# marcinp7/music-style-transfer

Hardware: AMD Instinct MI355X
Metric: style-transfer opt iters/sec (higher is better)
Workload: dtype f32; 1 GPU; one 30 s clip per GPU (BASELINE.json configs[1]): piano-roll C=4,R=16,T=4 (+percussion), full widths (980325 params), fwd+loss+bwd every step, Adam+StepLR every iter_size steps; clips_per_gpu=1, iter_size=2, hip_graph=True, graphs=one joint graph, accumulation=2 concurrent streams, launches_per_pass=72, parallelism=single GPU

## Files before the change

__graft_entry__.py:

```python
import os
import subprocess
import sys

ROOT = os.path.dirname(os.path.abspath(__file__))
PKG = os.path.join(ROOT, 'music-style-transfer_amd')
CSRC = os.path.join(PKG, 'csrc')
BUILD = os.path.join(PKG, 'build')
LIB = os.path.join(PKG, 'libmst_amd.so')
SOURCES = ['gemm', 'lstm', 'combine', 'notes', 'loss_optim', 'plan', 'audio', 'conv', 'lin']
for p in (ROOT, PKG):
    if p not in sys.path:
        sys.path.insert(0, p)


def _hipcc():
    for c in (os.environ.get('HIPCC'), '/opt/rocm/bin/hipcc', 'hipcc'):
        if c and (os.path.isabs(c) and os.path.exists(c) or not os.path.isabs(c)):
            return c
    raise RuntimeError('hipcc not found')


def _stale(target, deps):
    return not os.path.exists(target) or any(os.path.getmtime(d) > os.path.getmtime(target) for d in deps)


def build(force=False):
    os.makedirs(BUILD, exist_ok=True)
    hipcc = _hipcc()
    headers = [os.path.join(CSRC, 'mst_common.h'), os.path.join(CSRC, 'combine_body.h'), os.path.join(ROOT, 'include', 'mst_amd.h')]
    procs, objs = [], []
    for s in SOURCES:
        src, obj = os.path.join(CSRC, s + '.hip'), os.path.join(BUILD, s + '.o')
        objs.append(obj)
        if force or _stale(obj, [src] + headers):
            cmd = [hipcc, '--offload-arch=gfx950', '-O3', '-std=c++17', '-fPIC', '-c', src, '-o', obj]
            procs.append((s, subprocess.Popen(cmd, stdout=subprocess.PIPE, stderr=subprocess.STDOUT)))
    for s, p in procs:
        out, _ = p.communicate()
        if p.returncode:
            raise RuntimeError(f'hipcc failed on {s}.hip:\n{out.decode()}')
    if force or _stale(LIB, objs):
        subprocess.run([hipcc, '--offload-arch=gfx950', '-shared', '-fPIC', '-o', LIB] + objs, check=True)
    import style
    from style import _native
    _native.Native(LIB)


def smoke():
    import numpy as np
    import torch
    from oracle import style_oracle as so
    from tools.synth import synth_clip
    from style import _native as nat
    if not os.path.exists(LIB):
        build()
    assert torch.cuda.is_available(), 'smoke() needs cuda:0'
    dev = torch.device('cuda:0')
    native = nat.get()
    C, R, T = 2, 2, 4
    dims = nat.Dims(C=C, R=R, T=T, beat=64, bar=128, nrf=8, style=256, melody=8, rhythm=32, instr=51,
                    n_instruments=41, has_unpitched=1)
    table = native.param_table(dims)
    g = torch.Generator().manual_seed(0)
    flat = torch.zeros(native.param_floats(dims))
    named = {}
    for name, off, shape in table:
        n = int(np.prod(shape))
        fan = shape[1] if len(shape) > 1 else shape[0]
        flat[off:off + n] = (torch.rand(n, generator=g) * 2 - 1) / fan ** 0.5
        named[name] = flat[off:off + n].view(*shape).clone().requires_grad_(True)
    clip = synth_clip(5, C, R, T, True)
    _, ref_losses = so.iteration(named, clip)
    plan = native.plan(dims, dev)
    plan.set_inputs(mode=clip['mode'], bpm=clip['bpm'], instr=clip['instruments_features'],
                    used=clip['used_instruments'], bpm_target=float(clip['bpm_int']))
    params = flat.to(dev)
    gparams = torch.zeros_like(params)
    losses = torch.zeros(nat.N_LOSSES, device=dev)
    plan.train_iteration(params, gparams, clip['pitched'].to(dev), clip['unpitched'].to(dev), losses)
    torch.cuda.synchronize()
    got = losses.cpu()
    for i, k in enumerate(nat.LOSS_KEYS):
        assert abs(float(got[i]) - ref_losses[k]) < 1e-4, (k, float(got[i]), ref_losses[k])
    gref = torch.cat([(named[n].grad if named[n].grad is not None else torch.zeros_like(named[n])).reshape(-1)
                      for n, _, _ in table])
    err = float((gparams.cpu() - gref).norm() / gref.norm())
    assert err < 1e-4, err
    print(f'smoke ok: total loss {float(got[0]):.6f} (oracle {ref_losses["total"]:.6f}), grad rel-L2 {err:.2e}')


if __name__ == '__main__':
    build()
    print('built', LIB)
```

include/mst_amd.h:

```cpp
#ifndef MST_AMD_H
#define MST_AMD_H
#include <stdint.h>

#ifdef __cplusplus
extern "C" {
#endif

typedef enum {
    MST_OK = 0,
    MST_ERR_ARG = -1,
    MST_ERR_UNSUPPORTED = -2,
    MST_ERR_LAUNCH = -3,
    MST_ERR_ALLOC = -4,
} mst_status;

typedef struct {
    int32_t C, R, T;
    int32_t beat, bar, nrf;
    int32_t style, melody, rhythm;
    int32_t instr;
    int32_t n_instruments;
    int32_t has_unpitched;
    int32_t clips;
} mst_dims;
// ... 41 lines not shown

int32_t mst_forward(const mst_plan* p, int32_t stage_mask, const float* params, float* ws,
                    const float* pitched, const float* unpitched, mst_stream stream);

int32_t mst_backward(const mst_plan* p, int32_t stage_mask, const float* params, float* gparams,
                     float* ws, const float* pitched, const float* unpitched, mst_stream stream);
int32_t mst_zero_grads(const mst_plan* p, int32_t stage_mask, float* ws, mst_stream stream);
int64_t mst_plan_zero_floats(const mst_plan* p, int32_t stage_mask);

#define MST_LOSS_SAVED 512
int64_t mst_loss_scratch_floats(void);
int32_t mst_total_loss_fwd(const float* pitched_pred, const float* pitched_target, int64_t n_pitched_pos,
                           const float* unpitched_pred, const float* unpitched_target, int64_t n_unpitched_pos,
                           const float* instr_logits, const float* instr_target, int32_t n_instr,
                           const float* mode_logits, const float* mode_target,
                           const float* bpm_pred, const float* bpm_target,
                           int32_t normalize, float* losses, float* saved, float* scratch, mst_stream stream);
int32_t mst_total_loss_bwd(const float* pitched_pred, const float* pitched_target, int64_t n_pitched_pos,
                           const float* unpitched_pred, const float* unpitched_target, int64_t n_unpitched_pos,
                           const float* instr_logits, const float* instr_target, int32_t n_instr,
                           const float* mode_logits, const float* mode_target,
                           const float* bpm_pred, const float* bpm_target,
                           const float* saved, const float* grad_losses,
                           float* g_pitched, float* g_unpitched, float* g_instr, float* g_mode, float* g_bpm,
                           mst_stream stream);

int32_t mst_train_iteration(const mst_plan* p, const float* params, float* gparams, float* ws,
                            const float* pitched, const float* unpitched, float* losses, mst_stream stream);

#define MST_MAX_XCHG 8
int32_t mst_tiled_phase_count(const mst_plan* p);
int32_t mst_tiled_phase(const mst_plan* p, int32_t phase, const float* params, float* gparams, float* ws,
                        const float* pitched, const float* unpitched, float* losses, int32_t is_root,
                        mst_stream stream, int64_t xoff[MST_MAX_XCHG], int64_t xlen[MST_MAX_XCHG], int32_t* nx);

int32_t mst_adam_step(float* params, float* grads, float* exp_avg, float* exp_avg_sq, int64_t n,
                      float* state, double lr0, double beta1, double beta2, double eps,
                      int32_t step_size, double gamma, int32_t zero_grad, mst_stream stream);

int32_t mst_adam_step2(float* params, float* grads, float* grads2, float* exp_avg, float* exp_avg_sq, int64_t n,
                       float* state, double lr0, double beta1, double beta2, double eps,
                       int32_t step_size, double gamma, int32_t zero_grad, mst_stream stream);

#define MST_GUARD_WORDS 8
int64_t mst_grad_guard_scratch_bytes(int64_t n);
int32_t mst_grad_norm(const float* grads, const float* grads2 , int64_t n, void* scratch, float* norm,
                      mst_stream stream);
int32_t mst_grad_norms(const float* grads, const float* grads2 , const int64_t* offsets, const int64_t* lengths,
                       int32_t count, float* norms, mst_stream stream);
int32_t mst_adam_step_guarded(float* params, float* grads, float* grads2 , float* exp_avg, float* exp_avg_sq,
                              int64_t n, float* state, float* guard, void* scratch, double lr0, double beta1, double beta2,
                              double eps, int32_t step_size, double gamma, double max_norm ,
                              int32_t skip_nonfinite, int32_t zero_grad, mst_stream stream);

int32_t mst_hard_output(float* x, float* out, int64_t n_pos, int32_t nfeat, mst_stream stream);

int32_t mst_clip_scatter(const int32_t* cells, const float* feats, const int32_t* counts, int32_t capacity, int32_t n_clips,
                         int64_t n_cells, int32_t nfeat, float* out, mst_stream stream);

typedef struct { int32_t first, count, src_bars, r0; } mst_window;
int32_t mst_clip_window(const int32_t* cells, const float* feats, const mst_window* win, int32_t n_clips, int32_t channels,
                        int32_t bars, int64_t bar_cells, int32_t nfeat, float* out, mst_stream stream);

enum { MST_ROLL_NONZERO = 0, MST_ROLL_HARD = 1 };
int64_t mst_roll_slices(int64_t n_cells);
int32_t mst_roll_count(const float* x, int64_t n_cells, int32_t nfeat, int32_t mode, int32_t* ws, mst_stream stream);
int32_t mst_roll_compact(const float* x, int64_t n_cells, int32_t nfeat, int32_t mode, const int32_t* ws,
                         int64_t capacity, int32_t* cells, float* feats, mst_stream stream);

#define MST_METRIC_WORDS 8
int64_t mst_roll_metrics_scratch_bytes(int64_t n_groups, int64_t group_cells);
int32_t mst_roll_metrics(const float* pred, const float* target, int64_t n_groups, int64_t group_cells,
                         int32_t nfeat, void* scratch, double* out, mst_stream stream);

int64_t mst_eval_scratch_bytes(const mst_plan* p);
int32_t mst_eval_iteration(const mst_plan* p, const float* params, float* ws, const float* pitched,
                           const float* unpitched, float* losses, double* metrics, void* scratch, mst_stream stream);

int32_t mst_plan_step_count(const mst_plan* p, int32_t stage_mask, int32_t backward);
int32_t mst_plan_step_info(const mst_plan* p, int32_t stage_mask, int32_t backward, int32_t* info );
int32_t mst_plan_step_carried(const mst_plan* p, int32_t stage_mask, int32_t backward, int32_t* carried);
int32_t mst_plan_step_riders(const mst_plan* p, int32_t stage_mask, int32_t backward, int32_t* out);
int32_t mst_plan_zero_rides(const mst_plan* p);
int32_t mst_plan_step_gemms(const mst_plan* p, int32_t stage_mask, int32_t backward, int32_t step, int32_t* out, int32_t cap);
int32_t mst_plan_time_steps(const mst_plan* p, int32_t stage_mask, int32_t backward, const float* params,
                            float* gparams, float* ws, const float* pitched, const float* unpitched,
                            mst_stream stream, int32_t reps, float* ms, int32_t* kind, double* flops, double* bytes);

typedef struct mst_audio_plan mst_audio_plan;
mst_audio_plan* mst_audio_plan_create(int32_t n_fft , int32_t hop, int64_t n_samples, int32_t* status);
void mst_audio_plan_destroy(mst_audio_plan* p);
int32_t mst_audio_plan_info(const mst_audio_plan* p, int64_t out[6]);
int32_t mst_audio_stft(const mst_audio_plan* p, const float* audio, float* spec, float* mag, mst_stream stream);
int32_t mst_audio_gram(const mst_audio_plan* p, const float* feat, float* gram, float* ws, mst_stream stream);
int32_t mst_audio_style_iteration(const mst_audio_plan* p, float* x, const float* gram_style, float* grad, float* exp_avg,
                                  float* exp_avg_sq, float* state, float* ws, float* loss, double lr, mst_stream stream);

int32_t mst_debug_slab_columns_disjoint(int64_t off_x, int32_t width_x, int64_t off_y, int32_t width_y, int32_t ld);

const char* mst_version(void);

#ifdef __cplusplus
}
#endif
#endif
```

music-style-transfer_amd/csrc/gemm.hip:

```cpp
#include "combine_body.h"

__device__ __forceinline__ float act_fwd(int act, float z, int col) {
    if (act == ACT_LEAKY) return z > 0.f ? z : z * LEAKY;
    if (act == ACT_SIGOUT) { float s = 1.f / (1.f + expf(-z)); return col == 0 ? 6.f * s : s; }
    if (act == ACT_BPM) { float s = 1.f / (1.f + expf(-z)); return s * 150.f + 50.f; }
    return z;
}

__device__ __forceinline__ float act_bwd(int act, float y, int col) {
    if (act == ACT_LEAKY) return y > 0.f ? 1.f : LEAKY;
    if (act == ACT_SIGOUT) return col == 0 ? y * (1.f - y * (1.f / 6.f)) : y * (1.f - y);
    if (act == ACT_BPM) { float s = (y - 50.f) * (1.f / 150.f); return 150.f * s * (1.f - s); }
    return 1.f;
}

typedef const MST_GLOBAL_AS float* gcptr;
#define GEMM_PAD 1

template <int KIND>
__device__ __forceinline__ int off_of(const Operand& o, int i, int j, bool& ok) {
    if constexpr (KIND == OPK_DENSE) {
        return i * (int)o.si + j * (int)o.sj;
    } else if constexpr (KIND == OPK_ACTGRAD) {
        return o.transposed ? j * o.ld + i : i * o.ld + j;
    } else if constexpr (KIND == OPK_IM2COL) {
        const int p = i >> 3, oc = i & 7;
        const int f = j / (CONV_K * NPF), rem = j - f * (CONV_K * NPF);
        const int e = (NDEG * oc - CONV_PAD) * NPF + rem;
        ok = ok & (e >= 0) & (e < NPN * NPF);
        return p * (NF * NPN * NPF) + f * (NPN * NPF) + e;
    } else if constexpr (KIND == OPK_PERMW) {
        if (o.pb == CONV_K && o.pc == NPF) {
            constexpr int BC = CONV_K * NPF;
            const int a = i / BC, rem = i - a * BC;
            const int bb = rem / NPF, c = rem - bb * NPF;
            return j * o.ld + a * BC + c * CONV_K + bb;
        }
        if (o.pb == NUN && o.pc == NUF) {
            constexpr int BC = NUN * NUF;
            const int a = i / BC, rem = i - a * BC;
            const int bb = rem / NUF, c = rem - bb * NUF;
            return j * o.ld + a * BC + c * NUN + bb;
        }
        const int bc = o.pb * o.pc;
        const int a = i / bc, rem = i - a * bc;
        const int bb = rem / o.pc, c = rem - bb * o.pc;
        return j * o.ld + a * bc + c * o.pb + bb;
    } else {
        return (j >> 3) * (o.oc * NOCT) + i * NOCT + (j & 7);
    }
}

template <int OK>
__device__ __forceinline__ void store_out(const GemmDesc& d, float* cbase, const float* bias, int m, int n, int split, float acc) {
    const OutSpec& o = d.out;
    if constexpr (OK == OUT_STORE) {
        float v = acc;
        if (bias) v += o.bias_div > 0 ? bias[(unsigned)((m / o.bias_div) * o.bias_ld + n)] : bias[n];
        cbase[(unsigned)(m * o.ldc + n)] = act_fwd(o.act, v, n);
    } else if constexpr (OK == OUT_ACCUM) {
        float* c = cbase + (unsigned)(m * o.ldc + n);
        *c = o.first ? acc : *c + acc;
    } else if constexpr (OK == OUT_CONV) {
        cbase[(unsigned)((m >> 3) * o.ldc + n * NOCT + (m & 7))] = act_fwd(ACT_LEAKY, acc + bias[n], 0);
    } else if constexpr (OK == OUT_SLAB) {
        const unsigned idx = n < o.wcols ? (unsigned)(m * o.wcols + n) : (unsigned)(d.M * o.wcols + m);
        cbase[(int64_t)split * o.slab_stride + idx] = acc;
    } else {
        unsigned idx;
        if (n < o.wcols) {
            int a, bb, c, bc;
            if (o.pb == CONV_K && o.pc == NPF) { bc = CONV_K * NPF; a = n / (CONV_K * NPF); const int rem = n - a * (CONV_K * NPF); bb = rem / NPF; c = rem - bb * NPF; }
            else if (o.pb == NUN && o.pc == NUF) { bc = NUN * NUF; a = n / (NUN * NUF); const int rem = n - a * (NUN * NUF); bb = rem / NUF; c = rem - bb * NUF; }
            else { bc = o.pb * o.pc; a = n / bc; const int rem = n - a * bc; bb = rem / o.pc; c = rem - bb * o.pc; }
            idx = (unsigned)(m * o.wcols + a * bc + c * o.pb + bb);
        } else {
            idx = (unsigned)(d.M * o.wcols + m);
        }
        cbase[(int64_t)split * o.slab_stride + idx] = acc;
    }
}

template <int AK, int BKIND, int OK, int AKF, int BKF, int KD>
// ... 473 lines not shown
                    }
                }
            }
            const int n = tn * MF_BN + bn * 32 + (lane & 31);
            if ((ks == 0) & (tm * MF_BM + bm * 32 < M) & (tn * MF_BN + bn * 32 < N)) {
#pragma unroll
                for (int r = 0; r < 16; ++r) {
                    const int m = tm * MF_BM + bm * 32 + (r & 3) + 8 * (r >> 2) + 4 * (lane >> 5);
                    if (m < M && n < N) store_out<OK>(d, cbase, bias, m, n, split, acc[r]);
                }
            }
#pragma unroll
            for (int r = 0; r < 16; ++r) acc[r] = 0.f;
        }
        if (!more) break;
        t = nt; kt = nkt; buf ^= 1;
    }
}

__global__ __launch_bounds__(MF_THREADS, 4) void gemm_mfma_kernel(const GemmDesc* __restrict__ descs, const int* __restrict__ owner, int count, int blocks_per_clip, Bases b) {
    __shared__ float smem[2 * 2 * MF_KD * (MF_BM + GEMM_PAD)];
    float (*As)[MF_BM + GEMM_PAD] = reinterpret_cast<float (*)[MF_BM + GEMM_PAD]>(smem);
    float (*Bs)[MF_BN + GEMM_PAD] = reinterpret_cast<float (*)[MF_BN + GEMM_PAD]>(smem + MF_KD * (MF_BM + GEMM_PAD));
    const int clip = blockIdx.x / blocks_per_clip, lb = blockIdx.x - clip * blocks_per_clip;
    const int lo = owner[lb];
    const GemmDesc d = descs[clip * count + lo];
    const int local = lb - d.blk_begin;
    const int ntile = ((d.M + MF_BM - 1) / MF_BM) * ((d.N + MF_BN - 1) / MF_BN);
    const int run = d.run > 0 ? d.run : 1, nruns = (ntile + run - 1) / run;
    const int split = local / nruns, t_begin = (local - split * nruns) * run, t_end = min(ntile, t_begin + run);
    switch (d.variant) {
    case GV_LIN_FWD: gemm_fast_body<OPK_DENSE, OUT_STORE, 1, 1>(d, b, t_begin, t_end, split, smem); break;
    case GV_LIN_DW: gemm_fast_body<OPK_ACTGRAD, OUT_SLAB, 0, 0>(d, b, t_begin, t_end, split, smem); break;
    case GV_LIN_DW_PERM: gemm_fast_body<OPK_ACTGRAD, OUT_PERMW_SLAB, 0, 0>(d, b, t_begin, t_end, split, smem); break;
    case GV_LIN_DA: gemm_fast_body<OPK_ACTGRAD, OUT_ACCUM, 1, 0>(d, b, t_begin, t_end, split, smem); break;
    case GV_HH_DW: gemm_fast_body<OPK_DENSE, OUT_SLAB, 0, 0>(d, b, t_begin, t_end, split, smem); break;
    case GV_LIN_DA_RAW: gemm_fast_body<OPK_DENSE, OUT_ACCUM, 1, 0>(d, b, t_begin, t_end, split, smem); break;
    default:
        for (int tile = t_begin; tile < t_end; ++tile) {
            if (tile > t_begin) __syncthreads();
            if (d.variant == GV_LIN_FWD_PERM) gemm_mfma_body<OPK_DENSE, OPK_PERMW, OUT_STORE, 1, 1>(d, b, tile, split, As, Bs);
            else if (d.variant == GV_CONV_FWD) gemm_mfma_body<OPK_IM2COL, OPK_PERMW, OUT_CONV, 1, 1>(d, b, tile, split, As, Bs);
            else if (d.variant == GV_CONV_DW) {
                if (d.fold_rows) gemm_mfma_body<OPK_CONVGRAD, OPK_IM2COL, OUT_PERMW_SLAB, 1, 0, true>(d, b, tile, split, As, Bs);
                else gemm_mfma_body<OPK_CONVGRAD, OPK_IM2COL, OUT_PERMW_SLAB, 1, 0>(d, b, tile, split, As, Bs);
            }
        }
        break;
    }
}

int gemm_tile_edge(int mfma) { return mfma ? MF_BM : GEMM_BM; }
int gemm_blocks(const GemmDesc& g, int mfma) {
    const int edge = gemm_tile_edge(mfma);
    const int ntile = ((g.M + edge - 1) / edge) * ((g.N + edge - 1) / edge);
    const int run = (mfma && g.run > 1) ? g.run : 1;
    return ((ntile + run - 1) / run) * g.ksplit;
}

__device__ __forceinline__ void combine_rider(const CombineDesc d, const int cb, int kind, const Bases& b, float* smem) {
    constexpr int ROW = COMBINE_MAXC + 1;
    const int tid = threadIdx.x;
    if ((kind == COMB_RIDE_SUMSQ || kind == COMB_RIDE_REDUCE) && combine_site_small(d)) {
        if (cb != 0) return;
        kind = kind == COMB_RIDE_SUMSQ ? COMB_RIDE_SMALL_F : COMB_RIDE_SMALL_B;
    }
    if (kind == COMB_RIDE_SMALL_F) {
        combine_small_fwd_body<4>(d, tid, tid < 256, b, reinterpret_cast<float (*)[ROW]>(smem), smem + 4 * ROW);
    } else if (kind == COMB_RIDE_SMALL_B) {
        if (d.first) combine_small_bwd_body<4, true>(d, tid, tid < 256, b, smem, smem + ROW, reinterpret_cast<float (*)[ROW]>(smem + 2 * ROW));
        else combine_small_bwd_body<4, false>(d, tid, tid < 256, b, smem, smem + ROW, reinterpret_cast<float (*)[ROW]>(smem + 2 * ROW));
    } else {
        const int gi = tid >> 8, grp = cb * 4 + gi;
        float* slice = smem + gi * 5 * ROW;
        if (kind == COMB_RIDE_SUMSQ) combine_sumsq_body<4>(d, grp, tid & 255, grp < d.nblk, b, reinterpret_cast<float (*)[ROW]>(slice), slice + 4 * ROW);
        else combine_bwd_reduce_body<4>(d, grp, tid & 255, grp < d.nblk, b, reinterpret_cast<float (*)[ROW]>(slice), slice + 4 * ROW);
    }
}

template <int WV> __device__ __forceinline__ void gather_rows(const GatherDesc& d, const int blk, const int nblk, const Bases& b);
__device__ __forceinline__ void segred_group(const SegRedDesc* __restrict__ descs, const int members, const int clip, const int lb, const int t, const Bases& b);

__device__ __forceinline__ void gemm_rider_block(const GemmRiders& r, const int clip, int lb, const Bases& b, float* smem) {
    const int seg_blocks = (r.seg_groups + 3) >> 2, gat_blocks = r.gat_members * r.gat_blocks;
#pragma unroll
    for (int q = 0; q < 2; ++q) {
        const GemmRiders::Comb& cr = r.comb[q];
        const int comb_blocks = cr.sites * cr.blocks;
        if (lb < comb_blocks) {
            const int m = lb / cr.blocks;
            combine_rider(cr.descs[clip * cr.sites + m], lb - m * cr.blocks, cr.kind, b, smem);
            return;
        }
        lb -= comb_blocks;
    }
    if (lb < seg_blocks) {
        const int grp = lb * 4 + (threadIdx.x >> 8);
        if (grp < r.seg_groups) segred_group(r.segreds, r.seg_members, clip, grp, threadIdx.x & 255, b);
        return;
    }
    lb -= seg_blocks;
    if (lb < gat_blocks) {
        const int m = lb / r.gat_blocks;
        gather_rows<GATHER_RIDER_ROWS>(r.gathers[clip * r.gat_members + m], lb - m * r.gat_blocks, r.gat_blocks, b);
        return;
    }
    lb -= gat_blocks;
    if (lb < r.zero_chunks) {
        const ZeroChunk c = r.zero[lb];
        float* p = b.p[SP_GRAD] + (int64_t)clip * r.zero_stride + c.off;
        for (int i = threadIdx.x; i < c.len; i += GEMM_THREADS) p[i] = 0.f;
    }
}

__global__ __launch_bounds__(GEMM_THREADS) void gemm_kernel(const GemmDesc* __restrict__ descs, const int* __restrict__ owner, int count, int blocks_per_clip, int rider_blocks, Bases b, GemmRiders r) {
    constexpr int TILE_F = GEMM_BK * (GEMM_BM + GEMM_PAD), RED_F = (GEMM_THREADS / 64) * GEMM_BM * GEMM_BN;
    __shared__ float smem[(2 * TILE_F > RED_F) ? 2 * TILE_F : RED_F];
    float (*As)[GEMM_BM + GEMM_PAD] = reinterpret_cast<float (*)[GEMM_BM + GEMM_PAD]>(smem);
    float (*Bs)[GEMM_BN + GEMM_PAD] = reinterpret_cast<float (*)[GEMM_BN + GEMM_PAD]>(smem + TILE_F);
    const int clip = blockIdx.x / blocks_per_clip;
    int lb = blockIdx.x - clip * blocks_per_clip;
    if (lb < rider_blocks) {
        gemm_rider_block(r, clip, lb, b, smem);
        return;
    }
    lb -= rider_blocks;
    const int lo = owner[lb];
    const GemmDesc d = descs[clip * count + lo];
    const int local = lb - d.blk_begin;
    const int ntile = ((d.M + GEMM_BM - 1) / GEMM_BM) * ((d.N + GEMM_BN - 1) / GEMM_BN);
    const int tile = local % ntile, split = local / ntile;
#define GEMM_CASE(V, A_, B_, O_, AF_, BF_)                                                          \
    case (V) * 3 + 0: gemm_body<A_, B_, O_, AF_, BF_, 32>(d, b, tile, split, As, Bs); break;           \
    case (V) * 3 + 1: gemm_body<A_, B_, O_, AF_, BF_, 64>(d, b, tile, split, As, Bs); break;           \
    case (V) * 3 + 2: gemm_body<A_, B_, O_, AF_, BF_, 128>(d, b, tile, split, As, Bs); break;
    switch (d.variant * 3 + d.kdsel) {
        GEMM_CASE(GV_LIN_FWD, OPK_DENSE, OPK_DENSE, OUT_STORE, 1, 1)
        GEMM_CASE(GV_LIN_FWD_PERM, OPK_DENSE, OPK_PERMW, OUT_STORE, 1, 1)
        GEMM_CASE(GV_LIN_DW, OPK_ACTGRAD, OPK_DENSE, OUT_SLAB, 0, 0)
        GEMM_CASE(GV_LIN_DW_PERM, OPK_ACTGRAD, OPK_DENSE, OUT_PERMW_SLAB, 0, 0)
        GEMM_CASE(GV_LIN_DA, OPK_ACTGRAD, OPK_DENSE, OUT_ACCUM, 1, 0)
        GEMM_CASE(GV_CONV_FWD, OPK_IM2COL, OPK_PERMW, OUT_CONV, 1, 1)
        GEMM_CASE(GV_CONV_DW, OPK_CONVGRAD, OPK_IM2COL, OUT_PERMW_SLAB, 1, 0)
        GEMM_CASE(GV_HH_DW, OPK_DENSE, OPK_DENSE, OUT_SLAB, 0, 0)
        GEMM_CASE(GV_LIN_DA_RAW, OPK_DENSE, OPK_DENSE, OUT_ACCUM, 1, 0)
    default: break;
    }
#undef GEMM_CASE
}

int gemm_variant(const GemmDesc& g) {
    const int a = g.A.kind, bk = g.B.kind, o = g.out.kind;
    if (a == OPK_DENSE && bk == OPK_DENSE && o == OUT_STORE) return GV_LIN_FWD;
    if (a == OPK_DENSE && bk == OPK_PERMW && o == OUT_STORE) return GV_LIN_FWD_PERM;
    if (a == OPK_ACTGRAD && bk == OPK_DENSE && o == OUT_SLAB) return GV_LIN_DW;
    if (a == OPK_ACTGRAD && bk == OPK_DENSE && o == OUT_PERMW_SLAB) return GV_LIN_DW_PERM;
    if (a == OPK_ACTGRAD && bk == OPK_DENSE && o == OUT_ACCUM) return GV_LIN_DA;
    if (a == OPK_IM2COL && bk == OPK_PERMW && o == OUT_CONV) return GV_CONV_FWD;
    if (a == OPK_CONVGRAD && bk == OPK_IM2COL && o == OUT_PERMW_SLAB) return GV_CONV_DW;
    if (a == OPK_DENSE && bk == OPK_DENSE && o == OUT_SLAB) return GV_HH_DW;
    if (a == OPK_DENSE && bk == OPK_DENSE && o == OUT_ACCUM) return GV_LIN_DA_RAW;
    return -1;
}

int gemm_rider_blocks(const GemmRiders& r) { return r.comb[0].sites * r.comb[0].blocks + r.comb[1].sites * r.comb[1].blocks + (r.seg_groups + 3) / 4 + r.gat_members * r.gat_blocks + r.zero_chunks; }

int launch_gemm(const GemmDesc* dev_descs, const int* dev_owner, int members, int blocks_per_clip, int clips, int mfma, Bases b, hipStream_t s, const GemmRiders* riders) {
    if (members <= 0 || blocks_per_clip <= 0 || clips <= 0) return 0;
    GemmRiders r = riders ? *riders : GemmRiders{};
    if (mfma && gemm_rider_blocks(r)) return (int)hipErrorInvalidValue;
    blocks_per_clip += gemm_rider_blocks(r);
    if (mfma) hipLaunchKernelGGL(gemm_mfma_kernel, dim3(blocks_per_clip * clips), dim3(MF_THREADS), 0, s, dev_descs, dev_owner, members, blocks_per_clip, b);
    else hipLaunchKernelGGL(gemm_kernel, dim3(blocks_per_clip * clips), dim3(GEMM_THREADS), 0, s, dev_descs, dev_owner, members, blocks_per_clip, gemm_rider_blocks(r), b, r);
    return (int)hipGetLastError();
}

template <int WV>
__device__ __forceinline__ void gather_rows(const GatherDesc& d, const int blk, const int nblk, const Bases& b) {
    const int lane = threadIdx.x & 63, wv = (threadIdx.x >> 6) & (WV - 1);
    for (int row = blk * WV + wv; row < d.rows; row += nblk * WV) {
        unsigned t = (unsigned)row;
        int rc[4];
        rc[3] = t % (unsigned)d.d[3]; t /= (unsigned)d.d[3];
        rc[2] = t % (unsigned)d.d[2]; t /= (unsigned)d.d[2];
        rc[1] = t % (unsigned)d.d[1]; rc[0] = t / (unsigned)d.d[1];
        float* out = b.p[SP_WS] + d.out_off + (int64_t)row * d.K;
        if (d.sum) {
            for (int w = lane; w < d.K; w += 64) {
                float a = 0.f;
                for (int sIdx = 0; sIdx < d.nseg; ++sIdx) {
                    const Seg& sg = d.seg[sIdx];
                    const int srow = rc[0] * sg.s[0] + rc[1] * sg.s[1] + rc[2] * sg.s[2] + rc[3] * sg.s[3];
                    a += b.p[sg.space][sg.off + (int64_t)srow * sg.ld + w];
                }
                out[w] = a;
            }
            continue;
        }
        for (int sIdx = 0; sIdx < d.nseg; ++sIdx) {
            const Seg& sg = d.seg[sIdx];
            const int srow = rc[0] * sg.s[0] + rc[1] * sg.s[1] + rc[2] * sg.s[2] + rc[3] * sg.s[3];
            const float* src = b.p[sg.space] + sg.off + (int64_t)srow * sg.ld;
            for (int w = lane; w < sg.width; w += 64) out[sg.start + w] = src[w];
        }
    }
}

__global__ __launch_bounds__(256) void gather_kernel(const GatherDesc* __restrict__ descs, Bases b) {
    gather_rows<4>(descs[blockIdx.y], blockIdx.x, gridDim.x, b);
}

int launch_gather(const GatherDesc* dev, int count, int max_rows, Bases b, hipStream_t s) {
    if (count <= 0) return 0;
    int gx = (max_rows + 3) / 4;
    if (gx > 2048) gx = 2048;
    hipLaunchKernelGGL(gather_kernel, dim3(gx, count), dim3(256), 0, s, dev, b);
    return (int)hipGetLastError();
}

#define SEGRED_CHUNK 64
template <int E, int R>
__device__ __forceinline__ void segred_body(const SegRedDesc& d, const int item, const Bases& b) {
    const int wgrp = (d.width + E - 1) / E;
    if (item >= d.nidx * d.nchunk * wgrp) return;
    const int w = (item % wgrp) * E, ne = min(E, d.width - w);
    int t = item / wgrp;
    const int chunk = t % d.nchunk, idx = t / d.nchunk;
    int kc[4];
    t = idx;
#pragma unroll
    for (int q = 3; q >= 0; --q) { kc[q] = t % d.kd[q]; t /= d.kd[q]; }
    int rd[4], nred = 1;
#pragma unroll
    for (int q = 0; q < 4; ++q) { rd[q] = d.kd[q] == 1 ? d.d[q] : 1; nred *= rd[q]; }
    const int r_begin = chunk * SEGRED_CHUNK, r_end = min(nred, r_begin + SEGRED_CHUNK);
    int cr[4];
    t = r_begin;
#pragma unroll
    for (int q = 3; q >= 0; --q) { cr[q] = t % rd[q]; t /= rd[q]; }
    const float* src = b.p[SP_GRAD] + d.src_off + d.start + w;
    const float* ysrc = b.p[SP_WS] + d.y_off + d.start + w;
    const int64_t s3 = d.src_ld, s2 = s3 * d.d[3], s1 = s2 * d.d[2], s0 = s1 * d.d[1];
    const int64_t w3 = s2 - rd[3] * s3, w2 = s1 - rd[2] * s2, w1 = s0 - rd[1] * s1;
    int64_t roff = (kc[0] + cr[0]) * s0 + (kc[1] + cr[1]) * s1 + (kc[2] + cr[2]) * s2 + (kc[3] + cr[3]) * s3;
    auto offset = [&]() { return roff; };
    auto advance = [&]() {
        roff += s3;
        if (++cr[3] == rd[3]) { cr[3] = 0; roff += w3; if (++cr[2] == rd[2]) { cr[2] = 0; roff += w2; if (++cr[1] == rd[1]) { cr[1] = 0; roff += w1; ++cr[0]; } } }
// ... 162 lines not shown
```

music-style-transfer_amd/csrc/lstm.hip:

```cpp
#include "mst_common.h"

#define LSTM_ZS 8192
#define LSTM_MCH 32
__device__ __forceinline__ float sigm(float x) { return MST_FAST_RCP(1.f + MST_FAST_EXP(-x)); }
__device__ __forceinline__ float tanh_fast(float x) { return 2.f * sigm(2.f * x) - 1.f; }
__device__ __forceinline__ float wsum(float v) {
#pragma unroll
    for (int o = 32; o > 0; o >>= 1) v += __shfl_xor(v, o);
    return v;
}

typedef float lstm_f4 __attribute__((ext_vector_type(4)));
typedef float lstm_f4u __attribute__((ext_vector_type(4), aligned(4)));

template <bool REG>
__global__ __launch_bounds__(REG ? 256 : 1024) void lstm_fwd_kernel(const LstmDesc* __restrict__ descs, Bases b) {
    const LstmDesc d = descs[blockIdx.y];
    const int bi = blockIdx.x;
    if (bi >= d.B) return;
    const int H = d.H, G = 4 * d.H, tid = threadIdx.x;
    __shared__ float h_s[256];
    __shared__ float z_s[1024];
    __shared__ float zx_s[REG ? LSTM_ZS : 1];
    const int zchunk = REG ? LSTM_ZS / G : 1;
    const float* whh = b.p[SP_PAR] + d.whh_off;
    const float* zx = b.p[SP_WS] + d.zx_off;
    float* ws = b.p[SP_WS];
    float* tmp = b.p[SP_TMP];
    float w[REG ? 64 : 1];
    lstm_f4u wv[REG ? 16 : 1];
    const int wlast = max(G * H - 4, 0);
    if (REG && tid < G) {
#pragma unroll
        for (int k4 = 0; k4 < 16; ++k4) wv[k4] = *reinterpret_cast<const lstm_f4u*>(whh + min(tid * H + 4 * k4, wlast));
    }
    float bias[4] = {0.f, 0.f, 0.f, 0.f}, zq[4] = {0.f, 0.f, 0.f, 0.f};
    const int s0 = d.reverse ? d.S - 1 : 0;
    if (tid < H) {
#pragma unroll
        for (int q = 0; q < 4; ++q) {
            bias[q] = b.p[SP_PAR][d.bhh_off + q * H + tid];
            if (!REG) zq[q] = zx[((int64_t)bi * d.S + s0) * G + q * H + tid];
        }
    }
    auto fetch = [&](const int step) {
        const int cnt = min(zchunk, d.S - step);
        if (tid < G) {
            const MST_GLOBAL_AS float* zg = (const MST_GLOBAL_AS float*)zx + (int64_t)bi * d.S * G + tid;
            const int sstep = d.reverse ? -G : G;
            zg += (int64_t)(d.reverse ? d.S - 1 - step : step) * G;
            for (int i0 = 0; i0 < cnt; i0 += 16) {
                float t[16];
#pragma unroll
                for (int i = 0; i < 16; ++i) t[i] = zg[(int64_t)min(i0 + i, cnt - 1) * sstep];
#pragma unroll
                for (int i = 0; i < 16; ++i) MST_PIN(t[i]);
#pragma unroll
                for (int i = 0; i < 16; ++i) {
                    if (i0 + i < cnt) zx_s[(i0 + i) * G + tid] = t[i];
                }
            }
        }
    };
    if (REG) {
        fetch(0);
#pragma unroll
        for (int q = 0; q < 4; ++q) MST_PIN(bias[q]);
        if (tid < G) {
#pragma unroll
            for (int k4 = 0; k4 < 16; ++k4) {
                const int sh = tid * H + 4 * k4 - min(tid * H + 4 * k4, wlast);
                const lstm_f4u r = wv[k4];
                float v0 = r.x, v1 = r.y, v2 = r.z;
                v0 = sh == 1 ? r.y : v0; v0 = sh == 2 ? r.z : v0; v0 = sh == 3 ? r.w : v0;
                v1 = sh == 1 ? r.z : v1; v1 = sh == 2 ? r.w : v1;
                v2 = sh == 1 ? r.w : v2;
                w[4 * k4] = 4 * k4 < H ? v0 : 0.f; w[4 * k4 + 1] = 4 * k4 + 1 < H ? v1 : 0.f;
                w[4 * k4 + 2] = 4 * k4 + 2 < H ? v2 : 0.f; w[4 * k4 + 3] = 4 * k4 + 3 < H ? r.w : 0.f;
            }
        }
    }
    if (tid < 256) h_s[tid] = 0.f;
    float c = 0.f;
    for (int step = 0; step < d.S; ++step) {
        const int s = d.reverse ? d.S - 1 - step : step;
        const int64_t row = (int64_t)bi * d.S + s;
        float zn[4] = {0.f, 0.f, 0.f, 0.f};
        if (REG) {
            if (step % zchunk == 0 && step) {
                MST_LDS_BARRIER();
                fetch(step);
            }
        } else if (tid < H && step + 1 < d.S) {
            const int sn = d.reverse ? s - 1 : s + 1;
#pragma unroll
            for (int q = 0; q < 4; ++q) zn[q] = zx[((int64_t)bi * d.S + sn) * G + q * H + tid];
// ... 133 lines not shown
                for (int q = 0; q < 7; ++q) sv[q] = sv_s[(slot * 7 + q) * H + tid];
            } else if (step > 0) LSTM_LOAD(step - 1, nx)
            const float ig = sv[0], fg = sv[1], gg = sv[2], og = sv[3], tc = sv[4], cprev = sv[5];
            float dhr;
            if (chunked) {
                dhr = 0.f;
#pragma unroll
                for (int q = 0; q < 16; ++q) dhr += red_s[q * H + tid];
            } else dhr = (red_s[tid] + red_s[H + tid]) + (red_s[2 * H + tid] + red_s[3 * H + tid]);
            const float dh = sv[6] + dhr;
            const float dc = dc_next + dh * og * (1.f - tc * tc);
            const float dzi = dc * gg * ig * (1.f - ig);
            const float dzf = dc * cprev * fg * (1.f - fg);
            const float dzg = dc * ig * (1.f - gg * gg);
            const float dzo = dh * tc * og * (1.f - og);
            dc_next = dc * fg;
            dz_s[tid] = dzi; dz_s[H + tid] = dzf; dz_s[2 * H + tid] = dzg; dz_s[3 * H + tid] = dzo;
            float* gz = gr + d.gzx_off + row * G;
            gz[tid] = dzi; gz[H + tid] = dzf; gz[2 * H + tid] = dzg; gz[3 * H + tid] = dzo;
        }
        MST_LDS_BARRIER();
        float acc = 0.f;
        float cacc[4] = {0.f, 0.f, 0.f, 0.f};
        if (tid < G) {
            if (REG) {
                float a0 = 0.f, a1 = 0.f, a2 = 0.f, a3 = 0.f;
                const int base = part * H;
                float dv[64];
#pragma unroll
                for (int jj = 0; jj < 64; ++jj) dv[jj] = dz_s[min(base + jj, G - 1)];
                __builtin_amdgcn_sched_barrier(0);
#pragma unroll
                for (int jj = 0; jj < 64; jj += 4) {
                    a0 = fmaf(w[jj], dv[jj], a0);
                    a1 = fmaf(w[jj + 1], dv[jj + 1], a1);
                    a2 = fmaf(w[jj + 2], dv[jj + 2], a2);
                    a3 = fmaf(w[jj + 3], dv[jj + 3], a3);
                }
                acc = (a0 + a1) + (a2 + a3);
            } else {
                const float* wc = whh + (int64_t)part * H * H + kk;
                const float* dzp = dz_s + part * H;
                if (chunked) {
                    const int CH = H / 4;
                    float a[4][4];
#pragma unroll
                    for (int ci = 0; ci < 4; ++ci) { a[ci][0] = 0.f; a[ci][1] = 0.f; a[ci][2] = 0.f; a[ci][3] = 0.f; }
                    for (int jj = 0; jj < CH; jj += 4) {
#pragma unroll
                        for (int ci = 0; ci < 4; ++ci) {
#pragma unroll
                            for (int i = 0; i < 4; ++i) a[ci][i] = fmaf(wc[(int64_t)(ci * CH + jj + i) * H], dzp[ci * CH + jj + i], a[ci][i]);
                        }
                    }
#pragma unroll
                    for (int ci = 0; ci < 4; ++ci) cacc[ci] = (a[ci][0] + a[ci][1]) + (a[ci][2] + a[ci][3]);
                } else {
                    float a0 = 0.f, a1 = 0.f, a2 = 0.f, a3 = 0.f;
                    int jj = 0;
                    for (; jj + 4 <= H; jj += 4) {
                        a0 = fmaf(wc[(int64_t)jj * H], dzp[jj], a0);
                        a1 = fmaf(wc[(int64_t)(jj + 1) * H], dzp[jj + 1], a1);
                        a2 = fmaf(wc[(int64_t)(jj + 2) * H], dzp[jj + 2], a2);
                        a3 = fmaf(wc[(int64_t)(jj + 3) * H], dzp[jj + 3], a3);
                    }
                    for (; jj < H; ++jj) a0 = fmaf(wc[(int64_t)jj * H], dzp[jj], a0);
                    acc = (a0 + a1) + (a2 + a3);
                }
            }
        }
        if (!REG && tid < H) {
#pragma unroll
            for (int q = 0; q < 7; ++q) sv[q] = nx[q];
        }
        if (tid < G) {
            if (chunked) {
#pragma unroll
                for (int ci = 0; ci < 4; ++ci) red_s[(4 * part + ci) * H + kk] = cacc[ci];
            } else red_s[tid] = acc;
        }
        MST_LDS_BARRIER();
    }
#undef LSTM_LOAD
}


__global__ __launch_bounds__(1024) void lstm_fwd_wide_kernel(const LstmDesc* __restrict__ descs, Bases b) {
    const LstmDesc d = descs[blockIdx.y];
    const int bi = blockIdx.x;
    if (bi >= d.B) return;
    const int H = d.H, G = 4 * d.H, tid = threadIdx.x;
    const int KQ = ((H + 15) & ~15) / 4;
    __shared__ __attribute__((aligned(16))) float h_s[LSTM_WH];
    __shared__ __attribute__((aligned(16))) float z_s[4 * LSTM_WH];
    const MST_GLOBAL_AS float* zx = (const MST_GLOBAL_AS float*)(b.p[SP_WS] + d.zx_off) + (int64_t)bi * d.S * G;
    const MST_GLOBAL_AS lstm_f4* wt = (const MST_GLOBAL_AS lstm_f4*)(b.p[SP_TMP] + d.whht_off) + tid;
    MST_GLOBAL_AS float* ws = (MST_GLOBAL_AS float*)b.p[SP_WS];
    MST_GLOBAL_AS float* tmp = (MST_GLOBAL_AS float*)b.p[SP_TMP];
    float bias[4] = {0.f, 0.f, 0.f, 0.f}, zq[4] = {0.f, 0.f, 0.f, 0.f};
    const int s0 = d.reverse ? d.S - 1 : 0;
    if (tid < H) {
#pragma unroll
        for (int q = 0; q < 4; ++q) {
            bias[q] = b.p[SP_PAR][d.bhh_off + q * H + tid];
            zq[q] = zx[(int64_t)s0 * G + q * H + tid];
        }
    }
    h_s[tid] = 0.f;
    float c = 0.f;
    for (int step = 0; step < d.S; ++step) {
        const int s = d.reverse ? d.S - 1 - step : step;
        const int64_t row = (int64_t)bi * d.S + s;
        float zn[4] = {0.f, 0.f, 0.f, 0.f};
        if (tid < H && step + 1 < d.S) {
            const int sn = d.reverse ? s - 1 : s + 1;
#pragma unroll
            for (int q = 0; q < 4; ++q) zn[q] = zx[(int64_t)sn * G + q * H + tid];
        }
        MST_LDS_BARRIER();
        if (tid < H) {
            float a[4][4];
#pragma unroll
            for (int qq = 0; qq < 4; ++qq) { a[qq][0] = 0.f; a[qq][1] = 0.f; a[qq][2] = 0.f; a[qq][3] = 0.f; }
            for (int k = 0; k < KQ; k += 4) {
#pragma unroll
                for (int i = 0; i < 4; ++i) {
#pragma unroll
                    for (int qq = 0; qq < 4; ++qq) {
                        const int kk = qq * KQ + k + i;
                        const lstm_f4 w4 = wt[min(kk, H - 1) * H];
                        const float hv = h_s[kk];
                        a[qq][0] = fmaf(w4.x, hv, a[qq][0]); a[qq][1] = fmaf(w4.y, hv, a[qq][1]);
                        a[qq][2] = fmaf(w4.z, hv, a[qq][2]); a[qq][3] = fmaf(w4.w, hv, a[qq][3]);
                    }
                }
            }
            lstm_f4 z4;
            z4.x = (a[0][0] + a[1][0]) + (a[2][0] + a[3][0]); z4.y = (a[0][1] + a[1][1]) + (a[2][1] + a[3][1]);
            z4.z = (a[0][2] + a[1][2]) + (a[2][2] + a[3][2]); z4.w = (a[0][3] + a[1][3]) + (a[2][3] + a[3][3]);
            reinterpret_cast<lstm_f4*>(z_s)[tid] = z4;
        }
        MST_LDS_BARRIER();
        if (tid < H) {
            const float ig = sigm(z_s[tid] + zq[0] + bias[0]), fg = sigm(z_s[H + tid] + zq[1] + bias[1]);
            const float gg = tanh_fast(z_s[2 * H + tid] + zq[2] + bias[2]), og = sigm(z_s[3 * H + tid] + zq[3] + bias[3]);
            tmp[d.hprev_off + row * H + tid] = h_s[tid];
            c = fg * c + ig * gg;
            const float tc = tanh_fast(c);
            const float h = og * tc;
            tmp[d.tc_off + row * H + tid] = tc;
            MST_GLOBAL_AS float* g = tmp + d.gates_off + row * G;
            g[tid] = ig; g[H + tid] = fg; g[2 * H + tid] = gg; g[3 * H + tid] = og;
            tmp[d.c_off + row * H + tid] = c;
            ws[d.out_off + row * d.out_ld + tid] = h;
            h_s[tid] = h;
#pragma unroll
            for (int q = 0; q < 4; ++q) zq[q] = zn[q];
        }
    }
}

__global__ __launch_bounds__(1024) void lstm_bwd_wide_kernel(const LstmDesc* __restrict__ descs, Bases b) {
    const LstmDesc d = descs[blockIdx.y];
    const int bi = blockIdx.x;
    if (bi >= d.B) return;
    const int H = d.H, G = 4 * d.H, tid = threadIdx.x;
// ... 258 lines not shown
#ifdef HIPSIM
#define MST_COOP_LDS(name, n) static float name##_all[hipsim::COOP_MAXB][n]; float* name = name##_all[hipsim::coop_block()]
#define MST_COOP_LDS2(name, n, m) static float name##_all[hipsim::COOP_MAXB][n][m]; float (*name)[m] = name##_all[hipsim::coop_block()]
#define MST_LAUNCH_CORESIDENT(k, g, b, s, ...) hipsim::launch_coop((k), (g), (b), (s), __VA_ARGS__)
#else
#define MST_COOP_LDS(name, n) __shared__ __attribute__((aligned(16))) float name[n]
#define MST_COOP_LDS2(name, n, m) __shared__ float name[n][m]
#define MST_LAUNCH_CORESIDENT(k, g, b, s, ...) hipLaunchKernelGGL((k), (g), (b), 0, (s), __VA_ARGS__)
#endif

__global__ __launch_bounds__(256) void lstm_multi_fwd_kernel(const LstmDesc* __restrict__ descs, Bases b) {
    const LstmDesc d = descs[blockIdx.y];
    constexpr int H = LSTM_MH, G = 4 * H, HU = H / LSTM_NB, KQ = H / 4;
    const int wg = blockIdx.x, tid = threadIdx.x;
    const int row_l = tid >> 2, kq = tid & 3;
    const int gate = row_l / HU, u = row_l - gate * HU;
    const int j = gate * H + wg * HU + u;
    MST_COOP_LDS(h_s, H);
    MST_COOP_LDS(z_s, 4 * HU);
    const float* whh = b.p[SP_PAR] + d.whh_off;
    const float* zx = b.p[SP_WS] + d.zx_off;
    float* ws = b.p[SP_WS];
    float* tmp = b.p[SP_TMP];
    lstm_gran_t* xch = reinterpret_cast<lstm_gran_t*>(tmp + d.xch_off);
    int* status = reinterpret_cast<int*>(b.p[SP_WS] + d.status_off);
    bool dead = false;
    const unsigned fault = (d.multi == 2 && wg == 0) ? 0x10000u : 0u;
    float w[KQ];
#pragma unroll
    for (int i = 0; i < KQ / 4; ++i) {
        const float4 t4 = *reinterpret_cast<const float4*>(whh + (int64_t)j * H + kq * KQ + 4 * i);
        w[4 * i] = t4.x; w[4 * i + 1] = t4.y; w[4 * i + 2] = t4.z; w[4 * i + 3] = t4.w;
    }
    const int k = wg * HU + (tid < HU ? tid : 0);
    float bias[4] = {0.f, 0.f, 0.f, 0.f}, zq[4] = {0.f, 0.f, 0.f, 0.f};
    const int s0 = d.reverse ? d.S - 1 : 0;
    if (tid < HU) {
#pragma unroll
        for (int q = 0; q < 4; ++q) { bias[q] = b.p[SP_PAR][d.bhh_off + q * H + k]; zq[q] = zx[(int64_t)s0 * G + q * H + k]; }
    }
    float c = 0.f, hprev = 0.f;
    for (int step = 0; step < d.S; ++step) {
        const int s = d.reverse ? d.S - 1 - step : step;
        float zn[4] = {0.f, 0.f, 0.f, 0.f};
        if (tid < HU && step + 1 < d.S) {
            const int sn = d.reverse ? s - 1 : s + 1;
#pragma unroll
            for (int q = 0; q < 4; ++q) zn[q] = zx[(int64_t)sn * G + q * H + k];
        }
        if (tid < H) h_s[tid] = step == 0 ? 0.f : gran_wait(xch + ((step - 1) & 1) * H + tid, (unsigned)step, status, dead);
        __syncthreads();
        if (tid < HU) hprev = h_s[k];
        float a0 = 0.f, a1 = 0.f, a2 = 0.f, a3 = 0.f;
#pragma unroll
        for (int i = 0; i < KQ; i += 4) {
            const float4 h4 = *reinterpret_cast<const float4*>(h_s + kq * KQ + i);
            a0 = fmaf(w[i], h4.x, a0); a1 = fmaf(w[i + 1], h4.y, a1); a2 = fmaf(w[i + 2], h4.z, a2); a3 = fmaf(w[i + 3], h4.w, a3);
        }
        float zsum = (a0 + a1) + (a2 + a3);
        zsum += __shfl_xor(zsum, 1);
        zsum += __shfl_xor(zsum, 2);
        if (kq == 0) z_s[row_l] = zsum;
        __syncthreads();
        if (tid < HU) {
            const int64_t row = s;
            const float ig = sigm(z_s[tid] + zq[0] + bias[0]), fg = sigm(z_s[HU + tid] + zq[1] + bias[1]);
            const float gg = tanh_fast(z_s[2 * HU + tid] + zq[2] + bias[2]), og = sigm(z_s[3 * HU + tid] + zq[3] + bias[3]);
            c = fg * c + ig * gg;
            const float tc = tanh_fast(c);
            const float h = og * tc;
            gran_store(xch + (step & 1) * H + k, (unsigned)(step + 1) ^ (step == 0 ? fault : 0u), h);
            tmp[d.hprev_off + row * H + k] = hprev;
            tmp[d.tc_off + row * H + k] = tc;
            float* g = tmp + d.gates_off + row * G;
            g[k] = ig; g[H + k] = fg; g[2 * H + k] = gg; g[3 * H + k] = og;
            tmp[d.c_off + row * H + k] = c;
            ws[d.out_off + row * d.out_ld + k] = h;
#pragma unroll
            for (int q = 0; q < 4; ++q) zq[q] = zn[q];
        }
    }
}

#ifdef HIPSIM
#define LSTM_MULADD(a, b, c) ((a) * (b) + (c))
#else
#define LSTM_MULADD(a, b, c) __builtin_fmaf((a), (b), (c))
#endif

template <int N>
__device__ __forceinline__ void gran_wait_joint(const lstm_gran_t* g, unsigned tag, int* status, bool& dead, float (&v)[N]) {
#pragma unroll
    for (int i = 0; i < N; ++i) v[i] = __builtin_nanf("");
    if (dead) return;
    long long t0 = 0;
    unsigned need = (1u << N) - 1u;
    for (unsigned spin = 0;; ++spin) {
        lstm_gran_t x[N];
#pragma unroll
        for (int i = 0; i < N; ++i) {
            x[i] = 0;
            if ((need >> i) & 1u) x[i] = __hip_atomic_load(g + 256 * i, __ATOMIC_RELAXED, __HIP_MEMORY_SCOPE_AGENT);
        }
#pragma unroll
        for (int i = 0; i < N; ++i) {
            if (((need >> i) & 1u) && (unsigned)(x[i] >> 32) == tag) { v[i] = __uint_as_float((unsigned)x[i]); need &= ~(1u << i); }
        }
        if (!need) return;
        __builtin_amdgcn_s_sleep(1);
        if ((spin & 255u) == 255u) {
            if (__hip_atomic_load(status, __ATOMIC_RELAXED, __HIP_MEMORY_SCOPE_AGENT) != 0) break;
            const long long now = wall_clock64();
            if (spin == 255u) t0 = now;
            else if (now - t0 > LSTM_WAIT_TICKS) { __hip_atomic_fetch_or(status, MST_DEV_LSTM_TIMEOUT, __ATOMIC_RELAXED, __HIP_MEMORY_SCOPE_AGENT); break; }
        }
    }
    dead = true;
}

__global__ __launch_bounds__(256) void lstm_multi_bwd_kernel(const LstmDesc* __restrict__ descs, Bases b) {
    const LstmDesc d = descs[blockIdx.y];
    constexpr int H = LSTM_MH, G = 4 * H, HU = H / LSTM_NB, JQ = 16, JW = G / JQ;
    const int wg = blockIdx.x, tid = threadIdx.x;
    const int kk = tid & (HU - 1), jq = tid / HU;
    MST_COOP_LDS(dz_s, G);
    MST_COOP_LDS2(part_s, JQ, HU + 1);
    MST_COOP_LDS(sv_s, LSTM_MCH * 7 * HU);
    const float* whh = b.p[SP_PAR] + d.whh_off;
    const MST_GLOBAL_AS float* tmp = (const MST_GLOBAL_AS float*)b.p[SP_TMP];
    float* gr = b.p[SP_GRAD];
    const MST_GLOBAL_AS float* grg = (const MST_GLOBAL_AS float*)gr;
    int* status = reinterpret_cast<int*>(b.p[SP_WS] + d.status_off);
    bool dead = false;
    lstm_gran_t* xch = reinterpret_cast<lstm_gran_t*>(b.p[SP_TMP] + d.xch_off) + 2 * H;
    float w[JW];
#pragma unroll
    for (int i = 0; i < JW; ++i) w[i] = whh[(int64_t)(jq * JW + i) * H + wg * HU + kk];
    const int k = wg * HU + (tid < HU ? tid : 0);
    float dc_next = 0.f, dh_rec = 0.f;
#define LSTM_MLOAD(STEP, K, DST)                                                                        \
    {                                                                                                   \
        const int s_ = d.reverse ? d.S - 1 - (STEP) : (STEP);                                           \
        const int sp_ = d.reverse ? s_ + 1 : s_ - 1;                                                    \
        const MST_GLOBAL_AS float* g_ = tmp + d.gates_off + (int64_t)s_ * G;                            \
        DST[0] = g_[K]; DST[1] = g_[H + K]; DST[2] = g_[2 * H + K]; DST[3] = g_[3 * H + K];             \
        DST[4] = tmp[d.tc_off + (int64_t)s_ * H + K];                                                   \
        const float cp_ = tmp[d.c_off + (int64_t)((STEP) > 0 ? sp_ : s_) * H + K];       \
        DST[5] = (STEP) > 0 ? cp_ : 0.f;                                                                \
        DST[6] = grg[d.gout_off + (int64_t)s_ * d.out_ld + K];                                          \
    }
    auto stage = [&](const int step) {
        const int cnt = min(LSTM_MCH, step + 1), ku = wg * HU + kk;
#pragma unroll 4
        for (int i = jq; i < cnt; i += 64 / HU) {
            float t[7];
            LSTM_MLOAD(step - i, ku, t)
#pragma unroll
            for (int q = 0; q < 7; ++q) sv_s[(i * 7 + q) * HU + kk] = t[q];
        }
        MST_WAVE_SYNC();
    };
    if (tid < 64) stage(d.S - 1);
#pragma unroll
    for (int i = 0; i < JW; ++i) MST_PIN(w[i]);
    for (int step = d.S - 1; step >= 0; --step) {
        const int s = d.reverse ? d.S - 1 - step : step;
        const unsigned epoch = (unsigned)(d.S - step);
        const int par = (int)(epoch & 1);
        const int slot = (d.S - 1 - step) % LSTM_MCH;
        if (tid < 64 && slot == 0 && step != d.S - 1) stage(step);
        float dzi = 0.f, dzf = 0.f, dzg = 0.f, dzo = 0.f;
// ... 21 lines not shown
#pragma unroll
            for (int i = 0; i < G / 256; ++i) dz_s[tid + 256 * i] = dzv[i];
        }
        if (tid < HU) {
            float* gz = gr + d.gzx_off + (int64_t)s * G;
            gz[k] = dzi; gz[H + k] = dzf; gz[2 * H + k] = dzg; gz[3 * H + k] = dzo;
        }
        if (step == 0) break;
        __syncthreads();
        float a0 = 0.f, a1 = 0.f, a2 = 0.f, a3 = 0.f;
#pragma unroll
        for (int i = 0; i < JW; i += 4) {
            const float4 z4 = *reinterpret_cast<const float4*>(dz_s + jq * JW + i);
            a0 = fmaf(w[i], z4.x, a0); a1 = fmaf(w[i + 1], z4.y, a1); a2 = fmaf(w[i + 2], z4.z, a2); a3 = fmaf(w[i + 3], z4.w, a3);
        }
        part_s[jq][kk] = (a0 + a1) + (a2 + a3);
        __syncthreads();
        if (tid < HU) {
            float a = 0.f;
#pragma unroll
            for (int q = 0; q < JQ; ++q) a += part_s[q][tid];
            dh_rec = a;
        }
        __syncthreads();
    }
#undef LSTM_MLOAD
}

__global__ __launch_bounds__(256) void lstm_multi_clear_kernel(const LstmDesc* __restrict__ descs, Bases b) {
    const LstmDesc d = descs[blockIdx.y];
    if (!d.multi) return;
    float* x = b.p[SP_TMP] + d.xch_off;
    const int n = 2 * (2 * d.H + 8 * d.H);
    for (int i = blockIdx.x * 256 + threadIdx.x; i < n; i += gridDim.x * 256) x[i] = 0.f;
}

int lstm_multi_blocks_per_cu() {
#ifdef HIPSIM
    return 4;
#else
    int f = 0, w = 0;
    if (hipOccupancyMaxActiveBlocksPerMultiprocessor(&f, lstm_multi_fwd_kernel, 256, 0) != hipSuccess) return 0;
    if (hipOccupancyMaxActiveBlocksPerMultiprocessor(&w, lstm_multi_bwd_kernel, 256, 0) != hipSuccess) return 0;
    return f < w ? f : w;
#endif
}

__global__ __launch_bounds__(256) void lstm_transpose_kernel(const LstmDesc* __restrict__ descs, Bases b) {
    const LstmDesc d = descs[blockIdx.y];
    if (d.H <= 64 || d.multi) return;
    const int G = 4 * d.H, n = G * d.H;
    const float* w = b.p[SP_PAR] + d.whh_off;
    float* wt = b.p[SP_TMP] + d.whht_off;
    for (int e = blockIdx.x * 256 + threadIdx.x; e < n; e += gridDim.x * 256) {
        const int k = e / G, j = e - k * G;
        wt[e] = w[(int64_t)j * d.H + k];
    }
}

int launch_lstm_transpose(const LstmDesc* dev_descs, int count, int maxH, int multi, Bases b, hipStream_t s) {
    if (count <= 0 || maxH <= 64) return 0;
    if (multi) {
        hipLaunchKernelGGL(lstm_multi_clear_kernel, dim3(4, count), dim3(256), 0, s, dev_descs, b);
        return (int)hipGetLastError();
    }
    int nb = (4 * maxH * maxH + 255) / 256;
    if (nb > 256) nb = 256;
    hipLaunchKernelGGL(lstm_transpose_kernel, dim3(nb, count), dim3(256), 0, s, dev_descs, b);
    return (int)hipGetLastError();
}

static int block_for(int maxH) {
    if (lstm_band(maxH) == 2) return LSTM_WH;
    int t = (4 * maxH + 63) / 64 * 64;
    return t < 64 ? 64 : t;
}

#ifdef HIPSIM
static bool lstm_grouped(int, int maxB) { return maxB >= 2 * LSTM_NS; }
#else
static bool lstm_grouped(int count, int maxB) { return maxB >= 2 * LSTM_NS && (int64_t)count * maxB >= 2048; }
#endif

int launch_lstm_fwd(const LstmDesc* dev_descs, int count, int maxB, int maxH, int multi, Bases b, hipStream_t s) {
    if (count <= 0) return 0;
    if (multi) {
        MST_LAUNCH_CORESIDENT(lstm_multi_fwd_kernel, dim3(LSTM_NB, count), dim3(256), s, dev_descs, b);
        return (int)hipGetLastError();
    }
    if (maxH <= 64 && lstm_grouped(count, maxB))
        hipLaunchKernelGGL(lstm_fwd_group_kernel, dim3((maxB + LSTM_NS - 1) / LSTM_NS, count), dim3(256), 0, s, dev_descs, b);
    else if (maxH <= 64)
        hipLaunchKernelGGL((lstm_fwd_kernel<true>), dim3(maxB, count), dim3(block_for(maxH)), 0, s, dev_descs, b);
    else if (lstm_band(maxH) == 1)
        hipLaunchKernelGGL((lstm_fwd_kernel<false>), dim3(maxB, count), dim3(block_for(maxH)), 0, s, dev_descs, b);
    else
        hipLaunchKernelGGL(lstm_fwd_wide_kernel, dim3(maxB, count), dim3(block_for(maxH)), 0, s, dev_descs, b);
    return (int)hipGetLastError();
}

int launch_lstm_bwd(const LstmDesc* dev_descs, int count, int maxB, int maxH, int multi, Bases b, hipStream_t s) {
    if (count <= 0) return 0;
    if (multi) {
        MST_LAUNCH_CORESIDENT(lstm_multi_bwd_kernel, dim3(LSTM_NB, count), dim3(256), s, dev_descs, b);
        return (int)hipGetLastError();
    }
    if (maxH <= 64 && lstm_grouped(count, maxB))
        hipLaunchKernelGGL(lstm_bwd_group_kernel, dim3((maxB + LSTM_NS - 1) / LSTM_NS, count), dim3(256), 0, s, dev_descs, b);
    else if (maxH <= 64)
        hipLaunchKernelGGL((lstm_bwd_kernel<true>), dim3(maxB, count), dim3(block_for(maxH)), 0, s, dev_descs, b);
    else if (lstm_band(maxH) == 1)
        hipLaunchKernelGGL((lstm_bwd_kernel<false>), dim3(maxB, count), dim3(block_for(maxH)), 0, s, dev_descs, b);
    else
        hipLaunchKernelGGL(lstm_bwd_wide_kernel, dim3(maxB, count), dim3(block_for(maxH)), 0, s, dev_descs, b);
    return (int)hipGetLastError();
}
```

music-style-transfer_amd/csrc/mst_common.h:

```cpp
#pragma once
#include <hip/hip_runtime.h>
#include <stdint.h>

#include "../../include/mst_amd.h"

#ifndef MST_GLOBAL_AS
#define MST_GLOBAL_AS __attribute__((address_space(1)))
#endif
#ifndef MST_CONST_AS
#define MST_CONST_AS __attribute__((address_space(4)))
#endif
#ifndef MST_UNIFORM
#define MST_UNIFORM(x) __builtin_amdgcn_readfirstlane(x)
#endif
#ifndef MST_FAST_EXP
#define MST_FAST_EXP(x) __expf(x)
#define MST_FAST_RCP(x) __builtin_amdgcn_rcpf(x)
#define MST_PIN(x) asm volatile("" : "+v"(x))
#endif
#ifndef MST_PIN_SGPR
#if defined(__AMDGCN__)
#define MST_PIN_SGPR(p) asm volatile("" : "+s"(p))
#else
#define MST_PIN_SGPR(p) ((void)(p))
// ... 27 lines not shown

enum { SP_WS = 0, SP_PAR = 1, SP_GPAR = 2, SP_EXT0 = 3, SP_EXT1 = 4, SP_GRAD = 5, SP_TMP = 6, SP_COUNT = 7 };
enum { MST_BF_LOSS_FUSED = 1,
       MST_BF_ALL_STAGES = 2 };
struct Bases { float* p[SP_COUNT]; int32_t flags; };

enum { ACT_NONE = 0, ACT_LEAKY = 1, ACT_SIGOUT = 2, ACT_BPM = 3 };

enum { OPK_DENSE = 0, OPK_ACTGRAD = 2, OPK_IM2COL = 3, OPK_PERMW = 4, OPK_CONVGRAD = 5 };
#define MAX_SEG 6
struct Seg {
    int32_t space, ld, start, width;
    int64_t off;
    int32_t s[4];
};
struct Operand {
    int32_t kind;
    int32_t space;
    int64_t off;
    int64_t si, sj;
    int32_t ones_at;
    int32_t kfast;
    int32_t space2, ld, act, transposed;
    int64_t off2;
    int32_t oc;
    int32_t pb, pc;
};
enum { OUT_STORE = 0, OUT_ACCUM = 1, OUT_CONV = 2, OUT_SLAB = 3, OUT_PERMW_SLAB = 4 };
struct OutSpec {
    int32_t kind, space, ldc, act;
    int64_t off;
    int32_t bias_space;
    int64_t bias_off;
    int64_t slab_stride;
    int32_t first;
    int32_t wcols;
    int32_t pb, pc;
    int32_t bias_div, bias_ld;
};
struct GemmDesc {
    int32_t M, N, K, ksplit;
    int32_t variant;
    int32_t blk_begin;
    int32_t kdsel;
    int32_t run;
    int32_t fold_rows;
    int64_t acs, acs2, bcs;
    int32_t clip_rows;
    Operand A, B;
    OutSpec out;
};

struct GatherDesc {
    int32_t rows, K, nseg;
    int32_t sum;
    int32_t d[4];
    int64_t out_off;
    Seg seg[MAX_SEG];
};

struct SegRedDesc {
    int64_t src_off; int32_t src_ld; int32_t start, width;
    int64_t dst_off; int32_t dst_ld;
    int32_t d[4];
    int32_t s[4];
    int32_t nidx;
    int32_t kd[4];
    int32_t nchunk;
    int64_t part_off;
    int32_t blk_begin;
    int32_t first;
    int32_t act;
    int64_t y_off;
};

struct CombineDesc;
struct ZeroChunk;
enum { COMB_RIDE_NONE = 0, COMB_RIDE_SMALL_F, COMB_RIDE_SMALL_B, COMB_RIDE_SUMSQ, COMB_RIDE_REDUCE };
struct GemmRiders {
    const SegRedDesc* segreds; int32_t seg_members, seg_groups;
    const GatherDesc* gathers; int32_t gat_members, gat_blocks;
    struct Comb { const CombineDesc* descs; int32_t sites, blocks, kind; } comb[2];
    const ZeroChunk* zero; int32_t zero_chunks; int64_t zero_stride;
};

struct LstmDesc {
    int32_t B, S, H, reverse;
    int64_t zx_off;
    int64_t whh_off, bhh_off;
    int64_t out_off; int32_t out_ld;
    int64_t gates_off, c_off, hprev_off;
    int64_t tc_off;
    int64_t gout_off;
    int64_t gzx_off;
    int64_t whht_off;
    int32_t multi;
    int64_t xch_off;
    int64_t status_off;
};
#define LSTM_NB 12
#define LSTM_MH 192
#define LSTM_L2H 256
#define LSTM_WH 1024
static inline int lstm_band(int H) { return H <= 64 ? 0 : (H <= LSTM_L2H ? 1 : 2); }
static inline bool lstm_hidden_supported(int H) { return H >= 1 && H <= LSTM_WH; }

#define COMBINE_MAXC 32
#define COMBINE_MAXBLK 256
#define COMBINE_SMALL 4096
struct CombineDesc {
    int32_t Cn, rows, cols, ld;
    int64_t x_off, cs;
    int64_t out_off;
    int64_t stats_off;
    int64_t part_off;
    int64_t gx_off, gout_off;
    int32_t nblk;
    int32_t first;
};

struct NotesDesc {
    int32_t C, Q;
    int32_t W, CW, ML;
    int64_t oct_off, deg_off;
    int64_t rt_oct_off, rt_deg_off;
    int64_t it_oct_off, it_deg_off;
    int64_t x_off; int32_t x_space;
    int64_t mel_off, g_mel_off;
    int64_t wm_off;
    int64_t ml_off;
    int64_t wc_off, bc_off, wl_off, bl_off;
    int64_t out_off;
    int64_t g_out_off, g_oct_off, g_deg_off, g_ml_off;
    int64_t slab_off; int32_t slab_stride; int32_t nblk;
    int64_t itp_oct_off, itp_deg_off, loss_saved_off, loss_gl_off;
    int32_t fhn;
    int32_t nwc;
    int64_t part_off;
    int64_t stats_off;
};

struct ConvDesc {
    int32_t P, clips, OC, splits;
    int64_t rows_per_split;
    int64_t x1_off, clip_stride;
    int64_t wp_off;
    int64_t w_off, b_off;
    int64_t slab_off, slab_stride;
};
int launch_conv_prep(const ConvDesc& d, Bases b, hipStream_t s);
int launch_conv_fwd(const ConvDesc& d, Bases b, hipStream_t s);
int launch_conv_dw(const ConvDesc& d, Bases b, hipStream_t s);

typedef float mst_f32x16 __attribute__((ext_vector_type(16)));
template <int KT, bool M1 = true, bool N1 = true, int PA = 0, int PB = 0>
__device__ __forceinline__ void mst_mfma_ktile_2x2(const float (*As)[PA], const float (*Bs)[PB], int arow, int bcol, int l31, int kh,
                                                   mst_f32x16 (&acc)[2][2]) {
    float a0[2], a1[2], b0[2], b1[2];
    a0[0] = As[kh][arow + l31]; b0[0] = Bs[kh][bcol + l31];
    if (M1) a1[0] = As[kh][arow + 32 + l31];
    if (N1) b1[0] = Bs[kh][bcol + 32 + l31];
#pragma unroll
    for (int s = 0; s < KT / 2; ++s) {
        const int c = s & 1, n = c ^ 1;
        if (s + 1 < KT / 2) {
            const int k = 2 * (s + 1) + kh;
            a0[n] = As[k][arow + l31]; b0[n] = Bs[k][bcol + l31];
            if (M1) a1[n] = As[k][arow + 32 + l31];
            if (N1) b1[n] = Bs[k][bcol + 32 + l31];
        }
        __builtin_amdgcn_sched_barrier(0);
        acc[0][0] = __builtin_amdgcn_mfma_f32_32x32x2f32(a0[c], b0[c], acc[0][0], 0, 0, 0);
        if (N1) acc[0][1] = __builtin_amdgcn_mfma_f32_32x32x2f32(a0[c], b1[c], acc[0][1], 0, 0, 0);
        if (M1) acc[1][0] = __builtin_amdgcn_mfma_f32_32x32x2f32(a1[c], b0[c], acc[1][0], 0, 0, 0);
        if (M1 && N1) acc[1][1] = __builtin_amdgcn_mfma_f32_32x32x2f32(a1[c], b1[c], acc[1][1], 0, 0, 0);
        __builtin_amdgcn_sched_barrier(0);
    }
}


struct LinDesc {
    int32_t rows, K, N, act, xgrad, clips;
    int32_t x_space, x_ld; int64_t x_off, x_cs;
    int32_t y_ld; int64_t y_off, y_cs;
    int64_t gx_cs;
    int64_t w_off, b_off;
    int64_t slab_off, slab_stride, rows_per_split; int32_t splits;
    int32_t first[2];
};
int launch_lin_fwd(const LinDesc& d, Bases b, hipStream_t s);
int launch_lin_dx(const LinDesc& d, Bases b, int first, hipStream_t s);
int launch_lin_dw(const LinDesc& d, Bases b, hipStream_t s);
int lin_dw_tiles(const LinDesc& d);

struct RowLinDesc {
    int32_t rows, kin, nout, act, xgrad;
    int64_t x_off, y_off;
    int64_t w_off, b_off;
    int64_t slab_off; int32_t slab_stride, nblk;
    int32_t first;
};

struct CopyDesc { int64_t src_off, dst_off; int32_t na, nb, cols, src_sa, src_sb, dst_sa, dst_sb, first; };
struct FoldDesc { int32_t space, nrows, row_stride, ncols, col_stride, pad; int64_t part_off, sum_off ; };
int launch_copy_rows(const CopyDesc* dev, const CopyDesc& host, int backward, Bases b, hipStream_t s);
int launch_fold(const FoldDesc* dev, int spread, Bases b, hipStream_t s);
int launch_combine_phase(const CombineDesc* dev, int nblk, int which, Bases b, hipStream_t s, int count = 1, int mc4 = 0, int whole_small = 0);

struct SlabEntry { int64_t dst, src, stride; int32_t count, splits; int32_t reps; int64_t rep_stride; int32_t width, dst_ld; int32_t single;
                   int64_t base;  };
struct SlabBlock { int32_t entry, start; };

struct Sizes {
    int OC, PCE_IL, H, HB;
    int SE_L, SE_IL, SE_ML, SE_BL;
    int ME_BL, ME_BRL, ME_IL, ME_CW, MEL;
    int RH, PRE_BL, PRE_BRL, PRE_CL, PRE_IL, PRE_ML, PRE_BPL, URE_CL;
    int SIM_BL, NRF, SIM_SI, SIM_RI, SIM_SM, SIM_RM, SIM_SB, SIM_RB, NI;
    int PSA_SL, PSA_RL, PSA_IL, PSA_ML, USA_SL, USA_RL;
    int I, STYLE, BAR;
};
Sizes mst_sizes(const mst_dims& d);

enum { GV_LIN_FWD, GV_LIN_FWD_PERM, GV_LIN_DW, GV_LIN_DW_PERM, GV_LIN_DA, GV_CONV_FWD, GV_CONV_DW, GV_HH_DW, GV_LIN_DA_RAW };
int launch_gather(const GatherDesc* dev, int count, int max_rows, Bases b, hipStream_t s);
int gemm_variant(const GemmDesc& g);
int launch_gemm(const GemmDesc* dev_descs, const int* dev_owner, int members, int blocks_per_clip, int clips, int mfma, Bases b, hipStream_t s,
                const GemmRiders* riders = nullptr);
int gemm_rider_blocks(const GemmRiders& r);
int gemm_tile_edge(int mfma);
int gemm_blocks(const GemmDesc& g, int mfma);
int launch_segred(const SegRedDesc* dev_descs, int members, int blocks_per_clip, int clips, int stage2_blocks, Bases b, hipStream_t s);
int launch_segred2(const SegRedDesc* dev_descs, int count, int stage2_blocks, Bases b, hipStream_t s);
int launch_lstm_transpose(const LstmDesc* dev_descs, int count, int maxH, int multi, Bases b, hipStream_t s);
int launch_lstm_fwd(const LstmDesc* dev_descs, int count, int maxB, int maxH, int multi, Bases b, hipStream_t s);
int launch_lstm_bwd(const LstmDesc* dev_descs, int count, int maxB, int maxH, int multi, Bases b, hipStream_t s);
int lstm_multi_blocks_per_cu();
int launch_combine_fwd(const CombineDesc* dev_descs, int count, int max_nblk, int all_small, int mc4, Bases b, hipStream_t s);
int launch_combine_bwd(const CombineDesc* dev_descs, int count, int max_nblk, int all_small, int mc4, Bases b, hipStream_t s);
int launch_me_sumsq(const NotesDesc* dev, const NotesDesc& host, int count, Bases b, hipStream_t s);
int launch_me_notes_fwd(const NotesDesc* dev, const NotesDesc& host, int count, Bases b, hipStream_t s);
int launch_me_bwd_reduce(const NotesDesc* dev, const NotesDesc& host, int count, Bases b, hipStream_t s);
int launch_me_notes_bwd(const NotesDesc* dev, const NotesDesc& host, int count, Bases b, hipStream_t s);
int launch_psa_notes_fwd(const NotesDesc* dev, const NotesDesc& host, int count, Bases b, hipStream_t s);
int launch_psa_notes_bwd(const NotesDesc* dev, const NotesDesc& host, int count, Bases b, hipStream_t s);
int psa_bwd_waves(int C);
struct LossBatch { int32_t clips; int64_t ws, grad, tmp, ext0, ext1; };
int loss_fwd_partials(const float* pp, const float* pt, int64_t np, const float* up, const float* ut, int64_t nu, float* scratch,
                      hipStream_t s);
int loss_fwd_tail(int64_t np, int64_t nu, int has_u, const float* il, const float* it, int ni, const float* mlg, const float* mt,
                  const float* bp, const float* bt, int normalize, float* losses, float* saved, float* scratch, hipStream_t s,
                  float* gl_onehot, float* losses_out);
int loss_blocks(int64_t n);
int loss_fwd_batched(const float* pp, const float* pt, int64_t np, const float* up, const float* ut, int64_t nu, const float* il,
                     const float* it, int ni, const float* mlg, const float* mt, const float* bp, const float* bt, int normalize,
                     float* losses, float* saved, float* scratch, LossBatch lb, hipStream_t s,
                     float* gl_onehot ,
                     float* losses_out );
int loss_bwd_batched(const float* pp, const float* pt, int64_t np, const float* up, const float* ut, int64_t nu, const float* il,
                     const float* it, int ni, const float* mlg, const float* mt, const float* bp, const float* bt,
                     const float* saved, const float* gl, float* gp, float* gu, float* gi, float* gm, float* gb, LossBatch lb,
                     hipStream_t s, float info_scale = 1.f );
int launch_roll_metrics(const float* pred, const float* target, int64_t n_groups, int64_t group_cells, int nfeat, int gpc,
                        int64_t pred_cs, int64_t tgt_cs, void* scratch, hipStream_t s);
struct EvalMetricsArgs {
    const void* part_p; int64_t slices_p, cells_p;
    const void* part_u; int64_t slices_u, cells_u;
    int32_t C, ni;
    const float *il, *it, *mlg, *mt, *bp, *bt;
    int64_t ws_stride;
    double* out;
};
int launch_eval_metrics_finish(const EvalMetricsArgs& a, int clips, hipStream_t s);
bool rowlin_supported(int kin, int nout);
int launch_rowlin_fwd(const RowLinDesc* dev, const RowLinDesc& host, int count, Bases b, hipStream_t s);
int launch_rowlin_bwd(const RowLinDesc* dev, const RowLinDesc& host, int count, Bases b, hipStream_t s);
int launch_slab_reduce(const SlabEntry* dev, const SlabBlock* blocks, int nblocks, Bases b, hipStream_t s);
struct ZeroChunk { int64_t off; int32_t len; int32_t pad; };
int launch_zero(const ZeroChunk* dev, int nchunks, int clips, float* grad_base, int64_t clip_stride, hipStream_t s);
bool notes_widths_supported(int W, int CW, int ML);

#define GEMM_BM 32
#define GEMM_BN 32
#define GEMM_BK 128
#define GEMM_THREADS 1024
#define GATHER_RIDER_ROWS (GEMM_THREADS / 64)
```

music-style-transfer_amd/csrc/plan.hip:

```cpp
#include <cmath>
#include <cstdio>
#include <cstdlib>
#include <cstring>
#include <map>
#include <string>
#include <array>
#include <vector>

#include "mst_common.h"

#define MST_ALIGN_UP(n) (((n) + 63) / 64 * 64)

static int mean_size(double a, double b, double factor = 1.0) { return (int)std::ceil(((a + b) / 2.0) * factor); }

Sizes mst_sizes(const mst_dims& d) {
    Sizes z{};
    z.I = d.instr; z.STYLE = d.style; z.BAR = d.bar; z.H = d.beat; z.HB = d.bar / 2; z.RH = d.rhythm;
    z.MEL = d.melody; z.NRF = d.nrf; z.NI = d.n_instruments;
    z.OC = mean_size(NF * NPF, d.beat);
    z.PCE_IL = mean_size(d.instr, d.beat);
    z.SE_L = mean_size(d.bar, d.style);
    z.SE_IL = mean_size(d.instr, d.style, .25);
    z.SE_ML = mean_size(2, d.style, .1);
    z.SE_BL = mean_size(d.style, 1, .05);
// ... 115 lines not shown
    t.lin(m + ".scale_degree_linear", NPF * 6 * NDEG, z.PSA_SL + z.PSA_RL + z.PSA_IL);
    t.lin(m + ".melody_linear", z.PSA_ML, z.MEL);
    t.lin(m + ".linear", NPF, NPF * 6 + z.PSA_ML);
    m = "unpitched_style_applier";
    t.lin(m + ".style_linear", NF * z.USA_SL, z.STYLE);
    t.lin(m + ".rhythm_linear", z.USA_RL, z.RH);
    t.lin(m + ".notes_linear", NUN * NUF * 4, z.USA_SL + z.USA_RL);
    t.lin(m + ".linear", NUF, NUF * 4);
}

static bool widths_supported(const Sizes& z) {
    for (const int h : {z.H, z.HB, z.SE_L, z.SIM_BL, z.NRF})
        if (!lstm_hidden_supported(h)) return false;
    return notes_widths_supported(z.MEL, z.ME_CW, z.PSA_ML);
}

static bool dims_ok(const mst_dims* d) {
    return d && d->C >= 1 && d->C <= COMBINE_MAXC && d->C <= 24 && d->R >= 1 && d->T >= 1 && d->beat >= 1 && d->bar >= 2 &&
           d->bar % 2 == 0 && d->nrf >= 1 && d->style >= 1 && d->melody >= 1 && d->rhythm >= 1 && d->instr >= 1 &&
           d->n_instruments >= 1 && d->clips >= 0 && d->clips <= 4096;
}

extern "C" int32_t mst_param_count(const mst_dims* d) {
    if (!dims_ok(d)) return MST_ERR_ARG;
    ParamTable t; build_params(*d, mst_sizes(*d), t);
    return (int32_t)t.v.size();
}
extern "C" int64_t mst_param_floats(const mst_dims* d) {
    if (!dims_ok(d)) return MST_ERR_ARG;
    ParamTable t; build_params(*d, mst_sizes(*d), t);
    return t.top;
}
extern "C" int32_t mst_param_info(const mst_dims* d, int32_t i, char* name, int32_t cap, int64_t* off, int32_t* ndim,
                                  int32_t shape[3]) {
    if (!dims_ok(d) || !name || !off || !ndim || !shape) return MST_ERR_ARG;
    ParamTable t; build_params(*d, mst_sizes(*d), t);
    if (i < 0 || i >= (int)t.v.size()) return MST_ERR_ARG;
    const PInfo& p = t.v[i];
    snprintf(name, cap, "%s", p.name.c_str());
    *off = p.off; *ndim = p.ndim;
    for (int k = 0; k < 3; ++k) shape[k] = p.shape[k];
    return MST_OK;
}

struct T { int64_t off; int rows, cols, ld; };
struct SegIn { int space; int64_t off; int ld, width; int s[4]; bool grad; };
enum { K_GEMM, K_GATHER, K_SEGRED, K_LSTM_F, K_LSTM_B, K_COMB_F, K_COMB_B, K_ME_F, K_ME_B, K_PSA_F, K_PSA_B, K_LSTM_T, K_ROW_F, K_ROW_B,
       K_ME_SQ, K_ME_RED,
       K_COMB_F1, K_COMB_F2, K_COMB_B1, K_COMB_B2, K_COPY_F, K_COPY_B, K_FOLD, K_SPREAD, K_XCHG,
       K_GEMM_FOLD,
       K_CONV_P, K_CONV_F, K_CONV_W,
       K_LIN_F, K_LIN_A, K_LIN_W,
       K_COUNT };
enum { F_GEMM, F_GATHER, F_SEGRED, F_LSTM, F_COMB, F_NOTES, F_ROWLIN, F_COPY, F_FOLD, F_XCHG, F_CONV, F_LIN };
struct KindInfo { int kind, fam, sched, per_clip, merge; };
static constexpr KindInfo KINDS[] = {
    {K_GEMM, F_GEMM, 1, 1, 1},     {K_GATHER, F_GATHER, 1, 1, 1}, {K_SEGRED, F_SEGRED, 1, 1, 1}, {K_LSTM_F, F_LSTM, 1, 1, 1},
    {K_LSTM_B, F_LSTM, 1, 1, 1},   {K_COMB_F, F_COMB, 1, 1, 1},   {K_COMB_B, F_COMB, 1, 1, 1},   {K_ME_F, F_NOTES, 1, 1, 0},
    {K_ME_B, F_NOTES, 1, 1, 0},    {K_PSA_F, F_NOTES, 1, 1, 0},   {K_PSA_B, F_NOTES, 1, 1, 0},   {K_LSTM_T, F_LSTM, 1, 1, 1},
    {K_ROW_F, F_ROWLIN, 1, 1, 0},  {K_ROW_B, F_ROWLIN, 1, 1, 0},  {K_ME_SQ, F_NOTES, 1, 1, 0},   {K_ME_RED, F_NOTES, 1, 1, 0},
    {K_COMB_F1, F_COMB, 1, 1, 0},  {K_COMB_F2, F_COMB, 1, 1, 0},  {K_COMB_B1, F_COMB, 1, 1, 0},  {K_COMB_B2, F_COMB, 1, 1, 0},
    {K_COPY_F, F_COPY, 0, 0, 0},   {K_COPY_B, F_COPY, 0, 0, 0},   {K_FOLD, F_FOLD, 0, 0, 0},     {K_SPREAD, F_FOLD, 0, 0, 0},
    {K_XCHG, F_XCHG, 0, 0, 0},     {K_GEMM_FOLD, F_GEMM, 1, 0, 1}, {K_CONV_P, F_CONV, 0, 0, 0},  {K_CONV_F, F_CONV, 0, 0, 0},
    {K_CONV_W, F_CONV, 0, 0, 0},   {K_LIN_F, F_LIN, 0, 0, 0},     {K_LIN_A, F_LIN, 0, 0, 0},     {K_LIN_W, F_LIN, 0, 0, 0}};
static constexpr bool kinds_in_order(int i = 0) { return i == K_COUNT || (KINDS[i].kind == i && kinds_in_order(i + 1)); }
static_assert(sizeof(KINDS) / sizeof(KINDS[0]) == K_COUNT && kinds_in_order(), "KINDS[k] describes step kind k, for every k");

template <class D>
static int up(const std::vector<D>& v, D** dev) {
    *dev = nullptr;
    if (v.empty()) return 0;
    if (hipMalloc((void**)dev, v.size() * sizeof(D)) != hipSuccess) return MST_ERR_ALLOC;
    if (hipMemcpy(*dev, v.data(), v.size() * sizeof(D), hipMemcpyHostToDevice) != hipSuccess) return MST_ERR_ALLOC;
    return 0;
}
template <class D> struct DescTable {
    std::vector<D> host, sched;
    D* dev = nullptr;
    int upload() { return up(sched.empty() ? host : sched, &dev); }
    void release() { hipFree(dev); dev = nullptr; }
};

struct CombRide { int first = 0, sites = 0, nblk = 0, bwd = 0; };
struct Riders { int seg_first = 0, seg_members = 0, seg_groups = 0, seg_stage2 = 0, gat_first = 0, gat_members = 0, gat_rows = 0; CombRide comb[2]; };
struct Step { int kind, first, count, a, b, stage; int c = 0; int lvl = 0; int chain = -1; int signal = -1; int wait[3] = {-1, -1, -1};
              int carried = 0; Riders ride; };
struct Acc { int space; int64_t lo, hi; bool w; bool accum = false, dense = true; };
struct Op { int stage; std::vector<Step> fwd, bwd; };

static int stage_idx(int stage) { return stage == MST_STAGE_EXTRACT ? 0 : stage == MST_STAGE_INFO ? 1 : 2; }

struct mst_plan {
    mst_dims d; Sizes z; ParamTable pt;
    DescTable<GemmDesc> gemms; DescTable<GatherDesc> gathers; DescTable<SegRedDesc> segreds; DescTable<LstmDesc> lstms;
    DescTable<CombineDesc> combines; DescTable<NotesDesc> notes; DescTable<RowLinDesc> rowlins;
    DescTable<ConvDesc> convs; DescTable<LinDesc> lins; DescTable<CopyDesc> copies; DescTable<FoldDesc> folds;
    std::vector<SlabEntry> slabs[3];
    std::vector<Op> ops;
    std::vector<Step> sched[2];
    std::vector<Step> sched_all[2];
    const std::vector<Step>& list(int mask, int backward) const { return mask == MST_STAGE_ALL ? sched_all[backward ? 1 : 0] : sched[backward ? 1 : 0]; }
    std::vector<int> s_gemm_owner; int* d_gemm_owner = nullptr;
    std::map<std::string, T> named;
    int64_t act_top = 0, tmp_top = 0;
    SlabEntry* d_slabs[3] = {nullptr, nullptr, nullptr};
    std::vector<SlabBlock> slab_blocks[3]; SlabBlock* d_slab_blocks[3] = {nullptr, nullptr, nullptr};
    std::vector<SlabEntry> slabs_all; SlabEntry* d_slabs_all = nullptr;
    std::vector<SlabBlock> slab_blocks_all; SlabBlock* d_slab_blocks_all = nullptr;
    bool slabs_all_ok = false;
    T t_losses, t_saved, t_gl; int64_t loss_scratch = 0;
    std::vector<ZeroChunk> zero_stage[3], zero_all;
    ZeroChunk* d_zero_stage[3] = {nullptr, nullptr, nullptr}; ZeroChunk* d_zero_all = nullptr;
    int err = 0;
    mst_plan_options opt{};
    int mfma = 0;

    bool tiled() const { return opt.tile_rows > 0; }
    bool mixes() const { return !mfma && !tiled() && opt.branches != 1 && !opt.no_merge; }
    int mc4() const { return d.C <= 4 ? 1 : 0; }
    int Rl() const { return tiled() ? opt.tile_rows : d.R; }
    int P() const { return d.C * Rl() * d.T; }
    int Q() const { return Rl() * d.T; }
    struct Xchg { int space; int64_t off; int32_t len; };
    std::vector<Xchg> xchgs;
    bool tags_in_zero = false;
    int zero_ride = -1;
    void find_zero_ride();
    std::vector<ZeroChunk> zero_fwd; ZeroChunk* d_zero_fwd = nullptr;
    int64_t loss_sum_off = 0;
    int loss_fold[2] = {-1, -1};
    struct Phase { int what; int pass; int begin, end; int nx; int xchg[MST_MAX_XCHG]; };
    std::vector<Phase> phases;
    int K() const { return d.clips > 1 ? d.clips : 1; }
    static int device_cus() {
#ifdef HIPSIM
        return 16;
#else
        int dev = 0, cus = 0;
        if (hipGetDevice(&dev) != hipSuccess || hipDeviceGetAttribute(&cus, hipDeviceAttributeMultiprocessorCount, dev) != hipSuccess) return 0;
        return cus;
#endif
    }
    static int coresident_slots() {
        const int per_cu = lstm_multi_blocks_per_cu();
        return per_cu > 1 ? (per_cu - 1) * device_cus() : 0;
    }
    int64_t status_off = 0;
    enum { N_SIDE = 3, N_SETS = 4, N_EVENTS = 96 };
    struct SideSet { hipStream_t owner = nullptr; bool used = false; hipStream_t side[N_SIDE] = {}; hipEvent_t ev_fork = nullptr, ev_join[N_SIDE] = {}, ev[N_EVENTS] = {}; };
    mutable SideSet sides[N_SETS];
    bool branches = false;
    SideSet* side_set(hipStream_t main) const {
        for (SideSet& q : sides) if (q.used && q.owner == main) return &q;
        hipStreamCaptureStatus cs = hipStreamCaptureStatusNone;
        if (hipStreamIsCapturing(main, &cs) != hipSuccess || cs != hipStreamCaptureStatusNone) return nullptr;
        for (SideSet& q : sides) {
            if (q.used) continue;
            bool ok = hipEventCreateWithFlags(&q.ev_fork, hipEventDisableTiming) == hipSuccess;
            for (int i = 0; i < N_SIDE; ++i)
                ok = ok && hipStreamCreateWithFlags(&q.side[i], hipStreamNonBlocking) == hipSuccess &&
                     hipEventCreateWithFlags(&q.ev_join[i], hipEventDisableTiming) == hipSuccess;
            for (int i = 0; i < n_signals; ++i) ok = ok && hipEventCreateWithFlags(&q.ev[i], hipEventDisableTiming) == hipSuccess;
            if (!ok) return nullptr;
            q.used = true; q.owner = main;
            return &q;
        }
        return nullptr;
    }
    int64_t ext0_stride() const { return (int64_t)P() * NF * NPN * NPF; }
    int64_t ext1_stride() const { return (int64_t)Q() * NF * NUN * NUF; }
    int64_t shift(int space, int k) const {
        switch (space) {
        case SP_WS: case SP_GRAD: return (int64_t)k * act_top;
        case SP_TMP: return (int64_t)k * tmp_top;
        case SP_EXT0: return (int64_t)k * ext0_stride();
        case SP_EXT1: return (int64_t)k * ext1_stride();
        default: return 0;
        }
    }
    GemmDesc reloc(GemmDesc g, int k) const {
        for (Operand* o : {&g.A, &g.B}) {
            o->off += shift(o->space, k);
            if (o->kind == OPK_ACTGRAD || o->kind == OPK_CONVGRAD) o->off2 += shift(o->space2, k);
        }
        g.out.off += shift(g.out.space, k);
        if (g.out.bias_space >= 0) g.out.bias_off += shift(g.out.bias_space, k);
        return g;
    }
    GatherDesc reloc(GatherDesc g, int k) const {
        g.out_off += shift(SP_WS, k);
        for (int i = 0; i < g.nseg; ++i) g.seg[i].off += shift(g.seg[i].space, k);
        return g;
    }
    SegRedDesc reloc(SegRedDesc r, int k) const {
        r.src_off += shift(SP_GRAD, k); r.dst_off += shift(SP_GRAD, k); r.part_off += shift(SP_TMP, k); r.y_off += shift(SP_WS, k);
        return r;
    }
    LstmDesc reloc(LstmDesc l, int k) const {
// ... 937 lines not shown
        accesses(seq[i], acc[i]);
        for (int j = 0; j < i; ++j)
            if (level[j] >= level[i] && conflicts(acc[i], acc[j])) level[i] = level[j] + 1;
        if (level[i] > maxlevel) maxlevel = level[i];
    }
    std::vector<char> done(n, 0);
    for (int lv = 0; lv <= maxlevel; ++lv) {
        const size_t lv_begin = out.size();
        for (int i = 0; i < n; ++i) {
            if (done[i] || level[i] != lv) continue;
            const Step& s0 = seq[i];
            const KindInfo& ki = KINDS[s0.kind];
            const bool mergeable = !opt.no_merge && ki.merge, is_lstm = ki.fam == F_LSTM;
            Step m = s0; m.count = 0; m.lvl = lv;
            std::vector<int> members;
            for (int j = i; j < n; ++j) {
                if (done[j] || level[j] != lv) continue;
                const Step& s = seq[j];
                if (s.kind != s0.kind || (!across_stages && s.stage != s0.stage)) continue;
                if (is_lstm && lstm_band(s.b) != lstm_band(s0.b)) continue;
                if (is_lstm && j != i && (lstms.host[s.first].multi || lstms.host[s0.first].multi)) continue;
                if (j != i && !mergeable) continue;
                done[j] = 1;
                for (int q = 0; q < s.count; ++q) members.push_back(s.first + q);
                m.stage |= s.stage;
                if (s.a > m.a) m.a = s.a;
                if (s.b > m.b) m.b = s.b;
            }
            const bool shared_T = s0.kind == K_LSTM_T && !lstms.host[s0.first].multi;
            const int reps = ki.per_clip && !shared_T ? K() : 1;
            if (ki.sched)
                with_sched_table(ki.fam, [&](auto& t) {
                    m.first = (int)t.sched.size();
                    for (int k = 0; k < reps; ++k)
                        for (int idx : members) t.sched.push_back(reloc(t.host[idx], k));
                });
            m.count = (int)members.size() * reps;
            if (ki.fam == F_GEMM) {
                for (int q = 0; q < m.count; ++q) {
                    GemmDesc& g = gemms.sched[m.first + q];
                    g.variant = gemm_variant(g);
                    if (g.fold_rows) {
                        g.acs = shift(g.A.space, 1); g.acs2 = (g.A.kind == OPK_ACTGRAD || g.A.kind == OPK_CONVGRAD) ? shift(g.A.space2, 1) : 0; g.bcs = shift(g.B.space, 1);
                        if ((uint64_t)std::max(g.acs, std::max(g.acs2, g.bcs)) * (uint64_t)K() > 0xFFFFFFFFull) err = MST_ERR_UNSUPPORTED;
                    }
                    if (g.clip_rows) {
                        g.M = K();
                        if (g.A.kind == OPK_DENSE) g.A.si = shift(g.A.space, 1);
                        else g.A.ld = (int32_t)shift(g.A.space, 1);
                        g.out.ldc = (int32_t)shift(g.out.space, 1);
                        if ((uint64_t)act_top * (uint64_t)K() > 0x7FFFFFFFull) err = MST_ERR_UNSUPPORTED;
                    }
                    const int kr = (g.K + g.ksplit - 1) / g.ksplit;
                    g.kdsel = kr <= 32 ? 0 : (kr <= 64 ? 1 : 2);
                    g.run = (mfma && opt.gemm_run > 1) ? opt.gemm_run : 1;
                    if (g.variant < 0) err = MST_ERR_UNSUPPORTED;
                }
                const int nm = (int)members.size();
                int total = 0;
                m.c = (int)s_gemm_owner.size();
                for (int q = 0; q < nm; ++q) {
                    const int nb = gemm_blocks(gemms.sched[m.first + q], mfma);
                    for (int k = 0; k < reps; ++k) gemms.sched[m.first + k * nm + q].blk_begin = total;
                    total += nb;
                    s_gemm_owner.insert(s_gemm_owner.end(), nb, q);
                }
                m.a = total; m.b = nm;
            }
            if (m.kind == K_SEGRED) {
                const int nm = (int)members.size();
                int total = 0;
                for (int q = 0; q < nm; ++q) {
                    const SegRedDesc& r0 = segreds.sched[m.first + q];
                    for (int k = 0; k < reps; ++k) segreds.sched[m.first + k * nm + q].blk_begin = total;
                    total += (r0.nidx * r0.nchunk * r0.width + 255) / 256;
                }
                m.a = total;
            }
            out.push_back(m);
        }
        if (!mixes()) continue;
        for (size_t e = lv_begin; e < out.size(); ++e) {
            const bool comb = (out[e].kind == K_COMB_F || out[e].kind == K_COMB_B) && mc4();
            if (out[e].kind != K_GATHER && out[e].kind != K_SEGRED && !comb) continue;
            for (size_t c = lv_begin; c < out.size(); ++c) {
                Step& g = out[c];
                if (g.kind != K_GEMM || (!across_stages && g.stage != out[e].stage)) continue;
                const Step& s = out[e];
                if (s.kind == K_GATHER && !g.ride.gat_members) { g.ride.gat_first = s.first; g.ride.gat_members = s.count / K(); g.ride.gat_rows = s.a; }
                else if (s.kind == K_SEGRED && !g.ride.seg_members) { g.ride.seg_first = s.first; g.ride.seg_members = s.count / K(); g.ride.seg_groups = s.a; g.ride.seg_stage2 = s.b; }
                else if (comb && !g.ride.comb[s.b != 0].sites) g.ride.comb[s.b != 0] = CombRide{s.first, s.count / K(), s.a, s.kind == K_COMB_B};
                else continue;
                out[e].carried = 1;
                break;
            }
        }
    }
}

static bool covered(const std::vector<Acc>& have, int64_t lo, int64_t hi) {
    int64_t at = lo;
    bool moved = true;
    while (at < hi && moved) {
        moved = false;
        for (const Acc& a : have)
            if (a.lo <= at && a.hi > at) { at = a.hi; moved = true; }
    }
    return at >= hi;
}
static bool touches(const std::vector<Acc>& have, int64_t lo, int64_t hi) {
    for (const Acc& a : have) if (a.lo < hi && lo < a.hi) return true;
    return false;
}

void mst_plan::first_writers(std::vector<Step>& list, size_t begin, bool per_stage, std::vector<Acc>& zero) {
    std::vector<Acc> have;
    auto external = [&](const char* name) {
        auto it = named.find(name);
        if (it != named.end()) have.push_back(Acc{SP_GRAD, it->second.off, it->second.off + MST_ALIGN_UP((int64_t)it->second.rows * it->second.cols), true});
    };
    for (const char* nm : {"pitched_pred", "unpitched_pred", "instruments_pred", "mode_pred", "bpm_pred"}) external(nm);
    if (per_stage) for (const char* nm : {"style", "melody", "rhythm"}) external(nm);
    for (size_t si = begin; si < list.size(); ++si) {
        Step& m = list[si];
        const int reps = KINDS[m.kind].per_clip ? K() : 1, nm = m.count / reps;
        for (int q = 0; q < nm; ++q) {
            std::vector<Acc> acc;
            Step one = m; one.first = m.first + q; one.count = 1;
            accesses(one, acc, true);
            for (const Acc& a : acc) {
                if (a.space != SP_GRAD || a.w) continue;
                if (!covered(have, a.lo, a.hi)) { Acc z = a; z.w = true; z.space = m.stage; zero.push_back(z); have.push_back(a); }
            }
            int first = 0;
            bool accum = false;
            for (const Acc& a : acc) {
                if (a.space != SP_GRAD || !a.w) continue;
                if (!a.accum) { if (a.dense) have.push_back(a); continue; }
                accum = true;
                if (a.dense && !touches(have, a.lo, a.hi)) { first = 1; have.push_back(a); }
                else if (!covered(have, a.lo, a.hi)) { Acc z = a; z.space = m.stage; zero.push_back(z); have.push_back(a); }
            }
            if (!accum) continue;
            for (int k = 0, idx = m.first + q; k < reps; ++k, idx += nm) {
                switch (KINDS[m.kind].fam) {
                case F_GEMM: gemms.sched[idx].out.first = first; break;     case F_SEGRED: segreds.sched[idx].first = first; break;
                case F_COMB: combines.sched[idx].first = first; break;      case F_ROWLIN: rowlins.sched[idx].first = first; break;
                case F_COPY: copies.host[idx].first = first; break;         case F_LIN: lins.host[idx].first[per_stage ? 0 : 1] = first; break;
                }
            }
        }
    }
}

bool mst_plan::assign_streams(std::vector<Step>& L) {
    const int n = (int)L.size(), NS = 1 + N_SIDE;
    std::vector<std::vector<Acc>> acc(n);
    for (int i = 0; i < n; ++i) accesses(L[i], acc[i], true);
    auto dur = [&](const Step& st) {
        switch (st.kind) {
        case K_LSTM_F: case K_LSTM_B: return lstms.sched[st.first].multi ? 30.0 : 15.0;
        case K_ME_F: case K_ME_B: case K_PSA_F: case K_PSA_B: return 18.0;
        case K_GEMM: case K_GEMM_FOLD: return st.count > 8 ? 10.0 : 5.0;
        case K_SEGRED: return 9.0;
        default: return 5.0;
        }
    };
    const double EDGE_IN = 2.0, EDGE_X = 6.0;
    std::vector<double> fin(n, 0.0);
    std::vector<int> str(n, 0);
    double ready[1 + N_SIDE] = {};
    std::vector<std::array<int, 1 + N_SIDE>> clock(n);
    int tail[1 + N_SIDE]; for (int q = 0; q < NS; ++q) tail[q] = -1;
    for (int i = 0; i < n; ++i) {
// ... 200 lines not shown
    p->d = *d; p->z = mst_sizes(*d);
    if (p->d.clips < 1) p->d.clips = 1;
    build_params(*d, p->z, p->pt);
    p->build();
    if (!p->err) p->schedule();
    if (p->err) { *status = p->err; delete p; return nullptr; }
    int e = p->upload();
    if (e) { *status = e; mst_plan_destroy(p); return nullptr; }
    *status = MST_OK;
    return p;
}

extern "C" void mst_plan_destroy(mst_plan* p) {
    if (!p) return;
    p->gemms.release(); p->gathers.release(); p->segreds.release(); p->lstms.release(); p->combines.release(); p->notes.release();
    p->rowlins.release(); p->copies.release(); p->folds.release();
    hipFree(p->d_gemm_owner); hipFree(p->d_zero_all); hipFree(p->d_zero_fwd);
    for (int st = 0; st < 3; ++st) hipFree(p->d_zero_stage[st]);
    for (int s = 0; s < 3; ++s) { hipFree(p->d_slabs[s]); hipFree(p->d_slab_blocks[s]); }
    hipFree(p->d_slabs_all); hipFree(p->d_slab_blocks_all);
    for (mst_plan::SideSet& q : p->sides) {
        if (q.ev_fork) hipEventDestroy(q.ev_fork);
        for (int i = 0; i < mst_plan::N_SIDE; ++i) { if (q.ev_join[i]) hipEventDestroy(q.ev_join[i]); if (q.side[i]) hipStreamDestroy(q.side[i]); }
        for (hipEvent_t e : q.ev) if (e) hipEventDestroy(e);
    }
    delete p;
}

extern "C" int64_t mst_plan_workspace_floats(const mst_plan* p) { return p ? (int64_t)p->K() * (2 * p->act_top + p->tmp_top) : MST_ERR_ARG; }

extern "C" int32_t mst_plan_gemm_tile(const mst_plan* p) { return p ? (p->mfma ? 64 : 32) : MST_ERR_ARG; }

extern "C" int32_t mst_plan_layout(const mst_plan* p, int64_t out[4]) {
    if (!p || !out) return MST_ERR_ARG;
    out[0] = p->K(); out[1] = p->act_top; out[2] = p->tmp_top; out[3] = (int64_t)p->K() * p->act_top;
    return MST_OK;
}

extern "C" int32_t mst_plan_tensor(const mst_plan* p, const char* name, int64_t* off, int64_t* goff, int64_t* numel) {
    if (!p || !name) return MST_ERR_ARG;
    auto it = p->named.find(name);
    if (it == p->named.end()) return MST_ERR_ARG;
    if (off) *off = it->second.off;
    if (goff) *goff = (int64_t)p->K() * p->act_top + it->second.off;
    if (numel) *numel = (int64_t)it->second.rows * it->second.cols;
    return MST_OK;
}

extern "C" int32_t mst_plan_launch_count(const mst_plan* p, int32_t mask, int32_t backward) {
    if (!p) return MST_ERR_ARG;
    int n = 0;
    for (auto& s : p->list(mask, backward)) {
        if (!(s.stage & mask)) continue;
        const int stage2 = (((s.kind == K_COMB_F || s.kind == K_COMB_B) && s.b != 0) || (s.kind == K_SEGRED && s.b > 0)) ? 1 : 0;
        n += (s.carried ? 0 : 1) + stage2;
    }
    if (backward) for (int s = 0; s < 3; ++s) if ((mask >> s) & 1) n += 1;
    return n;
}

static Bases make_bases(const mst_plan* p, const float* params, float* gparams, float* ws, const float* pitched,
                        const float* unpitched) {
    Bases b;
    b.p[SP_WS] = ws; b.p[SP_PAR] = const_cast<float*>(params); b.p[SP_GPAR] = gparams;
    b.p[SP_EXT0] = const_cast<float*>(pitched); b.p[SP_EXT1] = const_cast<float*>(unpitched);
    b.p[SP_GRAD] = ws + (int64_t)p->K() * p->act_top; b.p[SP_TMP] = ws + 2 * (int64_t)p->K() * p->act_top;
    b.flags = 0;
    return b;
}

static int run_step(const mst_plan* p, const Step& s, const Bases& b, hipStream_t st, bool with_zero = false) {
    if (s.carried) return 0;
    switch (s.kind) {
    case K_GEMM: case K_GEMM_FOLD: {
        const Riders& q = s.ride;
        const int clips = s.count / s.b, gat_blocks = std::min(512, (q.gat_rows + GATHER_RIDER_ROWS - 1) / GATHER_RIDER_ROWS);
        GemmRiders r{p->segreds.dev + q.seg_first, q.seg_members, q.seg_groups, p->gathers.dev + q.gat_first, q.gat_members, gat_blocks};
        for (int large = 0; large < 2; ++large) {
            const CombRide& c = q.comb[large];
            if (!c.sites) continue;
            r.comb[large] = {p->combines.dev + c.first, c.sites, large ? (c.nblk + 3) / 4 : 1,
                             large ? (c.bwd ? COMB_RIDE_REDUCE : COMB_RIDE_SUMSQ) : (c.bwd ? COMB_RIDE_SMALL_B : COMB_RIDE_SMALL_F)};
        }
        if (with_zero) { r.zero = p->d_zero_all; r.zero_chunks = (int)p->zero_all.size(); r.zero_stride = p->act_top; }
        int e = launch_gemm(p->gemms.dev + s.first, p->d_gemm_owner + s.c, s.b, s.a, clips, p->mfma, b, st, &r);
        if (!e) e = launch_segred2(p->segreds.dev + q.seg_first, q.seg_members * clips, q.seg_stage2, b, st);
        if (!e && q.comb[1].sites)
            e = launch_combine_phase(p->combines.dev + q.comb[1].first, q.comb[1].nblk, q.comb[1].bwd ? 3 : 1, b, st, q.comb[1].sites * clips, 1, 1);
        return e;
    }
    case K_GATHER: return launch_gather(p->gathers.dev + s.first, s.count, s.a, b, st);
    case K_SEGRED: return launch_segred(p->segreds.dev + s.first, s.count / p->K(), s.a, p->K(), s.b, b, st);
    case K_LSTM_T: return launch_lstm_transpose(p->lstms.dev + s.first, s.count, s.b, p->lstms.sched[s.first].multi, b, st);
    case K_LSTM_F: return launch_lstm_fwd(p->lstms.dev + s.first, s.count, s.a, s.b, p->lstms.sched[s.first].multi, b, st);
    case K_LSTM_B: return launch_lstm_bwd(p->lstms.dev + s.first, s.count, s.a, s.b, p->lstms.sched[s.first].multi, b, st);
    case K_COMB_F: return launch_combine_fwd(p->combines.dev + s.first, s.count, s.a, s.b == 0 ? (p->mc4() ? 2 : 1) : 0, p->mc4(), b, st);
    case K_COMB_B: return launch_combine_bwd(p->combines.dev + s.first, s.count, s.a, s.b == 0 ? (p->mc4() ? 2 : 1) : 0, p->mc4(), b, st);
    case K_COMB_F1: return launch_combine_phase(p->combines.dev + s.first, s.a, 0, b, st, 1, p->mc4());
    case K_COMB_F2: return launch_combine_phase(p->combines.dev + s.first, s.a, 1, b, st, 1, p->mc4());
    case K_COMB_B1: return launch_combine_phase(p->combines.dev + s.first, s.a, 2, b, st, 1, p->mc4());
    case K_COMB_B2: return launch_combine_phase(p->combines.dev + s.first, s.a, 3, b, st, 1, p->mc4());
    case K_COPY_F: return launch_copy_rows(p->copies.dev + s.first, p->copies.host[s.first], 0, b, st);
    case K_COPY_B: return launch_copy_rows(p->copies.dev + s.first, p->copies.host[s.first], 1, b, st);
    case K_FOLD: return launch_fold(p->folds.dev + s.first, 0, b, st);
    case K_SPREAD: return launch_fold(p->folds.dev + s.first, 1, b, st);
    case K_XCHG: return MST_ERR_UNSUPPORTED;
    case K_LIN_F: case K_LIN_A: case K_LIN_W: {
        LinDesc l = p->lins.host[s.first];
        l.x_cs = p->shift(l.x_space, 1); l.y_cs = p->act_top; l.gx_cs = p->act_top;
        if (s.kind == K_LIN_F) return launch_lin_fwd(l, b, st);
        if (s.kind == K_LIN_W) return launch_lin_dw(l, b, st);
        return launch_lin_dx(l, b, l.first[(b.flags & MST_BF_ALL_STAGES) ? 1 : 0], st);
    }
    case K_CONV_P: { ConvDesc c = p->convs.host[s.first]; c.clip_stride = p->act_top; return launch_conv_prep(c, b, st); }
    case K_CONV_F: { ConvDesc c = p->convs.host[s.first]; c.clip_stride = p->act_top; return launch_conv_fwd(c, b, st); }
    case K_CONV_W: { ConvDesc c = p->convs.host[s.first]; c.clip_stride = p->act_top; return launch_conv_dw(c, b, st); }
    case K_ROW_F: return launch_rowlin_fwd(p->rowlins.dev + s.first, p->rowlins.sched[s.first], s.count, b, st);
    case K_ROW_B: return launch_rowlin_bwd(p->rowlins.dev + s.first, p->rowlins.sched[s.first], s.count, b, st);
    case K_ME_SQ: return launch_me_sumsq(p->notes.dev + s.first, p->notes.sched[s.first], s.count, b, st);
    case K_ME_RED: return launch_me_bwd_reduce(p->notes.dev + s.first, p->notes.sched[s.first], s.count, b, st);
    case K_ME_F: return launch_me_notes_fwd(p->notes.dev + s.first, p->notes.sched[s.first], s.count, b, st);
    case K_ME_B: return launch_me_notes_bwd(p->notes.dev + s.first, p->notes.sched[s.first], s.count, b, st);
    case K_PSA_F: return launch_psa_notes_fwd(p->notes.dev + s.first, p->notes.sched[s.first], s.count, b, st);
    case K_PSA_B: return launch_psa_notes_bwd(p->notes.dev + s.first, p->notes.sched[s.first], s.count, b, st);
    }
    return MST_ERR_ARG;
}

static int run_pass(const mst_plan* p, const std::vector<Step>& list, int mask, const Bases& b0, hipStream_t main, bool tags_cleared = false,
                    int zero_step = -1 ) {
    Bases b = b0;
    if (mask == MST_STAGE_ALL) b.flags |= MST_BF_ALL_STAGES;
    auto runs = [&](const Step& s) {
        if (!(s.stage & mask)) return false;
        if (tags_cleared && s.kind == K_LSTM_T && p->lstms.sched[s.first].multi) return false;
        return true;
    };
    mst_plan::SideSet* ss = (p->branches && mask == MST_STAGE_ALL) ? p->side_set(main) : nullptr;
    bool forked = false, used[mst_plan::N_SIDE] = {};
    for (auto& s : list) {
        if (!runs(s)) continue;
        hipStream_t st = main;
        if (ss) {
            if (s.chain > 0) {
                const int c = s.chain - 1;
                if (!forked) { if (hipEventRecord(ss->ev_fork, main) != hipSuccess) return MST_ERR_LAUNCH; forked = true; }
                if (!used[c]) { if (hipStreamWaitEvent(ss->side[c], ss->ev_fork, 0) != hipSuccess) return MST_ERR_LAUNCH; used[c] = true; }
                st = ss->side[c];
            }
            for (int w = 0; w < 3; ++w)
                if (s.wait[w] >= 0 && hipStreamWaitEvent(st, ss->ev[s.wait[w]], 0) != hipSuccess) return MST_ERR_LAUNCH;
        }
        int e = run_step(p, s, b, st, zero_step >= 0 && &s == &list[zero_step]);
        if (e) return e < 0 ? e : MST_ERR_LAUNCH;
        if (ss && s.signal >= 0 && hipEventRecord(ss->ev[s.signal], st) != hipSuccess) return MST_ERR_LAUNCH;
    }
    if (ss)
        for (int c = 0; c < mst_plan::N_SIDE; ++c)
            if (used[c] && (hipEventRecord(ss->ev_join[c], ss->side[c]) != hipSuccess || hipStreamWaitEvent(main, ss->ev_join[c], 0) != hipSuccess)) return MST_ERR_LAUNCH;
    return MST_OK;
}

extern "C" int32_t mst_forward(const mst_plan* p, int32_t mask, const float* params, float* ws, const float* pitched,
                               const float* unpitched, mst_stream stream) {
    if (!p || !params || !ws) return MST_ERR_ARG;
    if ((mask & MST_STAGE_EXTRACT) && (!pitched || (p->d.has_unpitched && !unpitched))) return MST_ERR_ARG;
    const Bases b = make_bases(p, params, nullptr, ws, pitched, unpitched);
    return run_pass(p, p->list(mask, 0), mask, b, (hipStream_t)stream);
}

extern "C" int32_t mst_plan_status(const mst_plan* p, float* ws, int32_t clear, int32_t* status, mst_stream stream) {
    if (!p || !ws || !status) return MST_ERR_ARG;
    if (hipStreamSynchronize((hipStream_t)stream) != hipSuccess) return MST_ERR_LAUNCH;
    int32_t word = 0;
    if (hipMemcpy(&word, ws + p->status_off, sizeof(word), hipMemcpyDeviceToHost) != hipSuccess) return MST_ERR_LAUNCH;
    *status = word;
    if (clear && word) {
        const int32_t zero = 0;
// ... 198 lines not shown
    }
    case K_CONV_F: case K_CONV_W: {
        const ConvDesc& c = p->convs.host[s.first];
        const double rows = (double)c.clips * c.P * NOCT, kk = NF * NPF * CONV_K;
        f = 2.0 * rows * c.OC * kk;
        b = 4.0 * (rows / NOCT * NF * NPN * NPF + rows * c.OC * (s.kind == K_CONV_F ? 1.0 : 2.0) + c.OC * kk);
        break;
    }
    case K_SEGRED:
        for (int i = 0; i < s.count; ++i) {
            const SegRedDesc& r = p->segreds.sched[s.first + i];
            const double rows = (double)r.d[0] * r.d[1] * r.d[2] * r.d[3];
            f += rows * r.width; b += 4.0 * (rows * r.width + 2.0 * r.nidx * r.width);
        }
        break;
    case K_LSTM_F: case K_LSTM_B:
        for (int i = 0; i < s.count; ++i) {
            const LstmDesc& l = p->lstms.sched[s.first + i];
            f += (double)l.B * l.S * (8.0 * l.H * l.H + 30.0 * l.H);
            b += 4.0 * ((double)l.B * l.S * 11.0 * l.H + 4.0 * l.H * l.H);
        }
        break;
    case K_COMB_F: case K_COMB_B:
        for (int i = 0; i < s.count; ++i) {
            const CombineDesc& c = p->combines.sched[s.first + i];
            const double n = (double)c.rows * c.cols;
            f += n * c.Cn * (s.kind == K_COMB_F ? 4.0 : 8.0);
            b += 4.0 * n * (s.kind == K_COMB_F ? 2.0 * c.Cn + 1 : 4.0 * c.Cn + 2);
        }
        break;
    case K_ROW_F: case K_ROW_B:
        for (int i = 0; i < s.count; ++i) {
            const RowLinDesc& r = p->rowlins.sched[s.first + i];
            const double mm = 2.0 * r.rows * r.kin * r.nout;
            f += s.kind == K_ROW_F ? mm : 2.0 * mm;
            b += 4.0 * r.rows * (s.kind == K_ROW_F ? r.kin + r.nout : 2.0 * r.kin + 2.0 * r.nout + (r.xgrad ? r.kin : 0));
        }
        break;
    case K_ME_SQ: case K_ME_F: case K_ME_RED: case K_ME_B: {
        const NotesDesc& n = p->notes.sched[s.first];
        const double pos = (double)n.C * n.Q * NF * NPN * s.count, mel = pos / n.C * n.W;
        const double per = 2.0 * n.W + 2.0 * n.CW * NPF + 2.0 * n.W * (n.W + n.CW);
        if (s.kind == K_ME_SQ) { f = pos * (per + 2.0 * n.W); b = 4.0 * pos * NPF; }
        else if (s.kind == K_ME_F) { f = pos * 2.0 * n.W; b = 4.0 * (pos * NPF + mel); }
        else if (s.kind == K_ME_RED) { f = pos * 2.0 * n.W; b = 4.0 * (pos * NPF + 2.0 * mel); }
        else { f = pos * per * 2.0; b = 4.0 * (pos * NPF + mel); }
        break;
    }
    case K_PSA_F: case K_PSA_B: {
        const NotesDesc& n = p->notes.sched[s.first];
        const double pos = (double)n.C * n.Q * NF * NPN * s.count;
        const double per = 2.0 * 30 + 2.0 * NPF * (30 + n.ML);
        f = pos * per * (s.kind == K_PSA_F ? 1.0 : 3.0);
        b = 4.0 * (pos * NPF * (s.kind == K_PSA_F ? 1.0 : 2.0) + (double)s.count * n.C * n.Q * NF * 450 * (s.kind == K_PSA_F ? 1.0 : 2.0) +
                   (double)s.count * n.Q * NF * NPN * n.ML * (s.kind == K_PSA_F ? 1.0 : 2.0));
        break;
    }
    }
    *flops = f; *bytes = b;
}

extern "C" int64_t mst_plan_zero_floats(const mst_plan* p, int32_t mask) {
    if (!p) return MST_ERR_ARG;
    int64_t n = 0;
    if ((mask & MST_STAGE_ALL) == MST_STAGE_ALL) { for (auto& c : p->zero_all) n += c.len; return n; }
    for (int s = 0; s < 3; ++s) if ((mask >> s) & 1) for (auto& c : p->zero_stage[s]) n += c.len;
    return n;
}

extern "C" int32_t mst_plan_step_carried(const mst_plan* p, int32_t mask, int32_t backward, int32_t* carried) {
    if (!p || !carried) return MST_ERR_ARG;
    int n = 0;
    for (auto& s : p->list(mask, backward))
        if (s.stage & mask) carried[n++] = (!s.carried || (s.kind != K_GATHER && s.kind != K_SEGRED)) ? 0 : ((s.kind == K_SEGRED && s.b > 0) ? 2 : 1);
    return n;
}

extern "C" int32_t mst_plan_step_riders(const mst_plan* p, int32_t mask, int32_t backward, int32_t* out) {
    if (!p || !out) return MST_ERR_ARG;
    int n = 0;
    for (auto& s : p->list(mask, backward)) {
        if (!(s.stage & mask)) continue;
        const bool two = (s.kind == K_SEGRED && s.b > 0) || ((s.kind == K_COMB_F || s.kind == K_COMB_B) && s.b != 0);
        out[n++] = !s.carried ? 0 : (two ? 2 : 1);
    }
    return n;
}

extern "C" int32_t mst_plan_zero_rides(const mst_plan* p) { return !p ? MST_ERR_ARG : (p->zero_ride >= 0 ? 1 : 0); }

extern "C" int32_t mst_plan_step_count(const mst_plan* p, int32_t mask, int32_t backward) {
    if (!p) return MST_ERR_ARG;
    int n = 0;
    for (auto& s : p->list(mask, backward)) if (s.stage & mask) ++n;
    return n;
}

extern "C" int32_t mst_plan_step_info(const mst_plan* p, int32_t mask, int32_t backward, int32_t* info ) {
    if (!p || !info) return MST_ERR_ARG;
    std::vector<const Step*> steps;
    for (auto& s : p->list(mask, backward)) if (s.stage & mask) steps.push_back(&s);
    int idx = 0;
    for (const Step* s : steps) {
        int32_t* o = info + 8 * idx++;
        o[0] = o[1] = o[2] = o[3] = 0; o[4] = s->count; o[5] = s->kind; o[6] = s->lvl; o[7] = s->chain;
        if (s->kind == K_GEMM || s->kind == K_GEMM_FOLD) { const GemmDesc& g = p->gemms.sched[s->first]; o[0] = g.M; o[1] = g.N; o[2] = g.K; o[3] = g.ksplit; }
        else if (KINDS[s->kind].fam == F_LIN) { const LinDesc& l = p->lins.host[s->first]; o[0] = l.rows; o[1] = l.N; o[2] = l.K; o[3] = l.splits; }
        else if (s->kind == K_LSTM_F || s->kind == K_LSTM_B) { const LstmDesc& l = p->lstms.sched[s->first]; o[0] = l.B; o[1] = l.S; o[2] = l.H; o[3] = l.multi; }
        else if (s->kind == K_GATHER) { const GatherDesc& g = p->gathers.sched[s->first]; o[0] = g.rows; o[1] = g.K; o[2] = g.nseg; }
        else if (s->kind == K_SEGRED) { const SegRedDesc& r = p->segreds.sched[s->first]; o[0] = s->a; o[1] = r.width; o[2] = r.d[0] * r.d[1] * r.d[2] * r.d[3]; }
        else if (s->kind == K_COMB_F || s->kind == K_COMB_B) { const CombineDesc& c = p->combines.sched[s->first]; o[0] = c.Cn; o[1] = c.rows; o[2] = c.cols; o[3] = c.nblk; }
    }
    return idx;
}

extern "C" int32_t mst_plan_step_gemms(const mst_plan* p, int32_t mask, int32_t backward, int32_t step, int32_t* out, int32_t cap) {
    if (!p || !out) return MST_ERR_ARG;
    int idx = 0;
    for (auto& s : p->list(mask, backward)) {
        if (!(s.stage & mask)) continue;
        if (idx++ != step) continue;
        if (s.kind != K_GEMM && s.kind != K_GEMM_FOLD) return 0;
        int n = 0;
        for (int q = 0; q < s.b && n < cap; ++q, ++n) {
            const GemmDesc& g = p->gemms.sched[s.first + q];
            int32_t* o = out + 6 * n;
            o[0] = g.M; o[1] = g.N; o[2] = g.K; o[3] = g.ksplit; o[4] = g.fold_rows; o[5] = gemm_blocks(g, p->mfma);
        }
        return n;
    }
    return MST_ERR_ARG;
}

extern "C" int32_t mst_plan_time_steps(const mst_plan* p, int32_t mask, int32_t backward, const float* params, float* gparams,
                                       float* ws, const float* pitched, const float* unpitched, mst_stream stream,
                                       int32_t reps, float* ms, int32_t* kind, double* flops, double* bytes) {
    if (!p || !params || !ws || !ms || !kind || !flops || !bytes || reps < 1) return MST_ERR_ARG;
    hipStream_t st = (hipStream_t)stream;
    Bases b = make_bases(p, params, gparams, ws, pitched, unpitched);
    if (backward && !p->tiled()) b.flags = MST_BF_LOSS_FUSED;
    if ((mask & MST_STAGE_ALL) == MST_STAGE_ALL) b.flags |= MST_BF_ALL_STAGES;
    hipEvent_t e0, e1;
    if (hipEventCreate(&e0) != hipSuccess || hipEventCreate(&e1) != hipSuccess) return MST_ERR_ALLOC;
    std::vector<const Step*> steps;
    for (auto& s : p->list(mask, backward)) if (s.stage & mask) steps.push_back(&s);
    int idx = 0;
    for (const Step* s : steps) {
        if (s->carried) {
            ms[idx] = 0.f; kind[idx] = s->kind;
            step_cost(p, *s, &flops[idx], &bytes[idx]);
            ++idx;
            continue;
        }
        run_step(p, *s, b, st);
        hipEventRecord(e0, st);
        for (int r = 0; r < reps; ++r) run_step(p, *s, b, st);
        hipEventRecord(e1, st);
        hipEventSynchronize(e1);
        float t = 0.f;
        hipEventElapsedTime(&t, e0, e1);
        ms[idx] = t / reps; kind[idx] = s->kind == K_GEMM_FOLD ? K_GEMM : s->kind;
        step_cost(p, *s, &flops[idx], &bytes[idx]);
        ++idx;
    }
    hipEventDestroy(e0); hipEventDestroy(e1);
    return idx;
}

extern "C" const char* mst_version(void) { return "mst_amd 0.1 (gfx950)"; }
// ... 1 lines not shown
```

music-style-transfer_amd/style/_native.py:

```python
import collections
import ctypes as C
import os

import torch

_HERE = os.path.dirname(os.path.abspath(__file__))
DEFAULT_LIB = os.path.join(os.path.dirname(_HERE), 'libmst_amd.so')

STAGE_EXTRACT, STAGE_INFO, STAGE_APPLY, STAGE_ALL = 1, 2, 4, 7
LOSS_SAVED = 512
LOSS_KEYS = [
    'total', 'channels_loss_total', 'channels_loss_pitched_total', 'channels_loss_pitched_notes_loss',
    'channels_loss_pitched_velocity_loss', 'channels_loss_pitched_duration_loss',
    'channels_loss_pitched_accidentals_loss', 'channels_loss_unpitched_total',
    'channels_loss_unpitched_notes_loss', 'channels_loss_unpitched_velocity_loss',
    'channels_loss_unpitched_duration_loss', 'song_info_loss_total', 'song_info_loss_instruments_loss',
    'song_info_loss_mode_loss', 'song_info_loss_bpm_loss',
]
N_LOSSES = len(LOSS_KEYS)


class MstError(RuntimeError):
    pass

# ... 11 lines not shown
                ('tile_rows', C.c_int32), ('lstm_flavour', C.c_int32), ('dense_flavour', C.c_int32), ('branches', C.c_int32)]


DEV_LSTM_TIMEOUT = 1
ROLL_NONZERO, ROLL_HARD = 0, 1
WINDOW_WORDS = 4
METRIC_WORDS = 8


def describe_status(word):
    parts = []
    if word & DEV_LSTM_TIMEOUT:
        parts.append('a granule of the multi-workgroup LSTM exchange did not arrive within 0.2 s (MST_DEV_LSTM_TIMEOUT): the '
                     'launch was not fully resident — something else occupied the GPU next to a batched plan; results since then '
                     'are NaN.  Plan option lstm_flavour=1 (MST_LSTM_FLAVOUR=1) takes the single-workgroup kernels')
    if word & ~DEV_LSTM_TIMEOUT:
        parts.append(f'unknown status bits {word & ~DEV_LSTM_TIMEOUT:#x}')
    return '; '.join(parts)


def options_from_env():
    ge = os.environ.get('MST_GEMM')
    if ge not in (None, '', 'mfma', 'valu'):
        raise MstError(f'MST_GEMM={ge!r}: expected mfma or valu')
    return dict(gemm_tile={'mfma': 64, 'valu': 32}.get(ge, 0), no_merge=int(bool(os.environ.get('MST_NO_MERGE'))),
                gemm_run=int(os.environ.get('MST_GEMM_RUN', '0')), lstm_flavour=int(os.environ.get('MST_LSTM_FLAVOUR', '0')),
                dense_flavour=int(os.environ.get('MST_DENSE_FLAVOUR', '0')), branches=int(os.environ.get('MST_BRANCHES', '0')))


_P = C.c_void_p
_SIGS = {
    'mst_param_count': (C.c_int32, [C.POINTER(Dims)]),
    'mst_param_floats': (C.c_int64, [C.POINTER(Dims)]),
    'mst_param_info': (C.c_int32, [C.POINTER(Dims), C.c_int32, C.c_char_p, C.c_int32, C.POINTER(C.c_int64),
                                   C.POINTER(C.c_int32), C.POINTER(C.c_int32 * 3)]),
    'mst_widths_supported': (C.c_int32, [C.POINTER(Dims)]),
    'mst_plan_create': (_P, [C.POINTER(Dims), C.POINTER(C.c_int32)]),
    'mst_plan_create_ex': (_P, [C.POINTER(Dims), C.POINTER(PlanOptions), C.POINTER(C.c_int32)]),
    'mst_plan_gemm_tile': (C.c_int32, [_P]),
    'mst_plan_destroy': (None, [_P]),
    'mst_plan_workspace_floats': (C.c_int64, [_P]),
    'mst_plan_tensor': (C.c_int32, [_P, C.c_char_p, C.POINTER(C.c_int64), C.POINTER(C.c_int64), C.POINTER(C.c_int64)]),
    'mst_plan_launch_count': (C.c_int32, [_P, C.c_int32, C.c_int32]),
    'mst_plan_layout': (C.c_int32, [_P, C.POINTER(C.c_int64 * 4)]),
    'mst_plan_status': (C.c_int32, [_P, _P, C.c_int32, C.POINTER(C.c_int32), _P]),
    'mst_debug_slab_columns_disjoint': (C.c_int32, [C.c_int64, C.c_int32, C.c_int64, C.c_int32, C.c_int32]),
    'mst_forward': (C.c_int32, [_P, C.c_int32, _P, _P, _P, _P, _P]),
    'mst_backward': (C.c_int32, [_P, C.c_int32, _P, _P, _P, _P, _P, _P]),
    'mst_zero_grads': (C.c_int32, [_P, C.c_int32, _P, _P]),
    'mst_plan_zero_floats': (C.c_int64, [_P, C.c_int32]),
    'mst_loss_scratch_floats': (C.c_int64, []),
    'mst_total_loss_fwd': (C.c_int32, [_P, _P, C.c_int64, _P, _P, C.c_int64, _P, _P, C.c_int32, _P, _P, _P, _P,
                                       C.c_int32, _P, _P, _P, _P]),
    'mst_total_loss_bwd': (C.c_int32, [_P, _P, C.c_int64, _P, _P, C.c_int64, _P, _P, C.c_int32, _P, _P, _P, _P,
                                       _P, _P, _P, _P, _P, _P, _P, _P]),
    'mst_train_iteration': (C.c_int32, [_P, _P, _P, _P, _P, _P, _P, _P]),
    'mst_tiled_phase_count': (C.c_int32, [_P]),
    'mst_tiled_phase': (C.c_int32, [_P, C.c_int32, _P, _P, _P, _P, _P, _P, C.c_int32, _P, C.POINTER(C.c_int64 * 8), C.POINTER(C.c_int64 * 8),
                        C.POINTER(C.c_int32)]),
    'mst_adam_step': (C.c_int32, [_P, _P, _P, _P, C.c_int64, _P, C.c_double, C.c_double, C.c_double, C.c_double,
                                  C.c_int32, C.c_double, C.c_int32, _P]),
    'mst_adam_step2': (C.c_int32, [_P, _P, _P, _P, _P, C.c_int64, _P, C.c_double, C.c_double, C.c_double, C.c_double,
                                   C.c_int32, C.c_double, C.c_int32, _P]),
    'mst_grad_guard_scratch_bytes': (C.c_int64, [C.c_int64]),
    'mst_grad_norm': (C.c_int32, [_P, _P, C.c_int64, _P, _P, _P]),
    'mst_grad_norms': (C.c_int32, [_P, _P, _P, _P, C.c_int32, _P, _P]),
    'mst_adam_step_guarded': (C.c_int32, [_P, _P, _P, _P, _P, C.c_int64, _P, _P, _P, C.c_double, C.c_double, C.c_double, C.c_double,
                                          C.c_int32, C.c_double, C.c_double, C.c_int32, C.c_int32, _P]),
    'mst_hard_output': (C.c_int32, [_P, _P, C.c_int64, C.c_int32, _P]),
    'mst_clip_scatter': (C.c_int32, [_P, _P, _P, C.c_int32, C.c_int32, C.c_int64, C.c_int32, _P, _P]),
    'mst_clip_window': (C.c_int32, [_P, _P, _P, C.c_int32, C.c_int32, C.c_int32, C.c_int64, C.c_int32, _P, _P]),
    'mst_roll_slices': (C.c_int64, [C.c_int64]),
    'mst_roll_count': (C.c_int32, [_P, C.c_int64, C.c_int32, C.c_int32, _P, _P]),
    'mst_roll_compact': (C.c_int32, [_P, C.c_int64, C.c_int32, C.c_int32, _P, C.c_int64, _P, _P, _P]),
    'mst_roll_metrics_scratch_bytes': (C.c_int64, [C.c_int64, C.c_int64]),
    'mst_roll_metrics': (C.c_int32, [_P, _P, C.c_int64, C.c_int64, C.c_int32, _P, _P, _P]),
    'mst_eval_scratch_bytes': (C.c_int64, [_P]),
    'mst_eval_iteration': (C.c_int32, [_P, _P, _P, _P, _P, _P, _P, _P, _P]),
    'mst_plan_step_count': (C.c_int32, [_P, C.c_int32, C.c_int32]),
    'mst_plan_step_info': (C.c_int32, [_P, C.c_int32, C.c_int32, _P]),
    'mst_plan_step_carried': (C.c_int32, [_P, C.c_int32, C.c_int32, _P]),
    'mst_plan_step_riders': (C.c_int32, [_P, C.c_int32, C.c_int32, _P]),
    'mst_plan_zero_rides': (C.c_int32, [_P]),
    'mst_plan_step_gemms': (C.c_int32, [_P, C.c_int32, C.c_int32, C.c_int32, _P, C.c_int32]),
    'mst_plan_time_steps': (C.c_int32, [_P, C.c_int32, C.c_int32, _P, _P, _P, _P, _P, _P, C.c_int32, _P, _P, _P, _P]),
    'mst_audio_plan_create': (_P, [C.c_int32, C.c_int32, C.c_int64, C.POINTER(C.c_int32)]),
    'mst_audio_plan_destroy': (None, [_P]),
    'mst_audio_plan_info': (C.c_int32, [_P, C.POINTER(C.c_int64 * 6)]),
    'mst_audio_stft': (C.c_int32, [_P, _P, _P, _P, _P]),
    'mst_audio_gram': (C.c_int32, [_P, _P, _P, _P, _P]),
    'mst_audio_style_iteration': (C.c_int32, [_P, _P, _P, _P, _P, _P, _P, _P, _P, C.c_double, _P]),
    'mst_version': (C.c_char_p, []),
}


def ptr(t):
    if t is None:
        return None
    if t.dtype != torch.float32 or not t.is_contiguous():
        raise MstError('mst_amd kernels take contiguous float32 tensors')
    return t.data_ptr()


def check(status, what):
    if status != 0:
        names = {-1: 'MST_ERR_ARG', -2: 'MST_ERR_UNSUPPORTED', -3: 'MST_ERR_LAUNCH', -4: 'MST_ERR_ALLOC'}
        raise MstError(f'{what} failed: {names.get(status, status)}')


class Native:
    def __init__(self, path=None):
        path = path or DEFAULT_LIB
        if not os.path.exists(path):
            raise MstError(
                f'{path} not found: the HIP library has not been built. Run `python -c "import __graft_entry__ as g; '
                f'g.build()"` (hipcc --offload-arch=gfx950). There is no CPU fallback.')
        self.path = path
        self.lib = C.CDLL(path)
        for name, (res, args) in _SIGS.items():
            fn = getattr(self.lib, name)
            fn.restype, fn.argtypes = res, args
        self._plans = collections.OrderedDict()
        self._plan_cap = int(os.environ.get('MST_PLAN_CACHE', '16'))

    def param_table(self, dims):
        n = self.lib.mst_param_count(C.byref(dims))
        if n <= 0:
            raise MstError('bad dims')
        out = []
        buf = C.create_string_buffer(256)
        off, nd, shp = C.c_int64(), C.c_int32(), (C.c_int32 * 3)()
        for i in range(n):
            check(self.lib.mst_param_info(C.byref(dims), i, buf, 256, C.byref(off), C.byref(nd), C.byref(shp)), 'mst_param_info')
            out.append((buf.value.decode(), off.value, tuple(shp[k] for k in range(nd.value))))
        return out

    def param_floats(self, dims):
        return self.lib.mst_param_floats(C.byref(dims))

    def clip_scatter(self, cells, feats, counts, out, n_cells, nfeat, n_clips=1, capacity=None, stream=None):
        if capacity is None:
            capacity = cells.numel() // n_clips
        addr = lambda t: t if t is None or isinstance(t, int) else t.data_ptr()
        check(self.lib.mst_clip_scatter(addr(cells), addr(feats), addr(counts), int(capacity), int(n_clips), int(n_cells), int(nfeat),
                                        addr(out), stream), 'mst_clip_scatter')

    def clip_window(self, cells, feats, win, out, n_clips, channels, bars, bar_cells, nfeat, stream=None):
        addr = lambda t: t if t is None or isinstance(t, int) else t.data_ptr()
        check(self.lib.mst_clip_window(addr(cells), addr(feats), addr(win), int(n_clips), int(channels), int(bars), int(bar_cells),
                                       int(nfeat), addr(out), stream), 'mst_clip_window')

    def roll_slices(self, n_cells):
        n = self.lib.mst_roll_slices(int(n_cells))
        if n <= 0:
            raise MstError(f'mst_roll_slices({n_cells}): need 1 <= n_cells < 2**31')
        return n

    def roll_count(self, x, n_cells, nfeat, mode, ws, stream=None):
        addr = lambda t: t if t is None or isinstance(t, int) else t.data_ptr()
        check(self.lib.mst_roll_count(addr(x), int(n_cells), int(nfeat), int(mode), addr(ws), stream), 'mst_roll_count')

    def roll_compact(self, x, n_cells, nfeat, mode, ws, capacity, cells, feats, stream=None):
        addr = lambda t: t if t is None or isinstance(t, int) else t.data_ptr()
        check(self.lib.mst_roll_compact(addr(x), int(n_cells), int(nfeat), int(mode), addr(ws), int(capacity), addr(cells), addr(feats),
                                        stream), 'mst_roll_compact')

# ... 81 lines not shown

    def view(self, name, shape=None, ws=None, clip=0):
        off, _, n = self.slot(name)
        off += clip * self.clip_stride
        t = (self.ws if ws is None else ws)[off:off + n]
        return t.view(*shape) if shape is not None else t

    def grad(self, name, shape=None, ws=None, clip=0):
        _, goff, n = self.slot(name)
        goff += clip * self.clip_stride
        t = (self.ws if ws is None else ws)[goff:goff + n]
        return t.view(*shape) if shape is not None else t

    def set_inputs(self, mode=None, bpm=None, instr=None, used=None, bpm_target=None, ws=None, clip=0):
        for name, t in (('mode', mode), ('bpm', bpm), ('instr', instr), ('used_instruments', used), ('bpm_target', bpm_target)):
            if t is not None:
                self.view(name, ws=ws, clip=clip).copy_(torch.as_tensor(t, dtype=torch.float32).reshape(-1), non_blocking=True)

    def status(self, ws=None, clear=True):
        word = C.c_int32()
        check(self.lib.mst_plan_status(self.handle, ptr(self.ws if ws is None else ws), int(bool(clear)), C.byref(word),
                                       current_stream(self.device)), 'mst_plan_status')
        return word.value

    def check_status(self, ws=None):
        word = self.status(ws)
        if word:
            raise MstError('device status: ' + describe_status(word))

    def _touch(self, ws):
        if self.branches and self.device.type == 'cuda' and torch.cuda.is_current_stream_capturing():
            raise MstError('a plan made with branches=1 cannot run under torch.cuda.graph capture; capture needs branches=0')
        ws = self.ws if ws is None else ws
        self._touched[id(ws)] = ws
        return ws

    def check_touched(self):
        touched, self._touched = self._touched, {}
        for ws in touched.values():
            self.check_status(ws)

    def launch_count(self, mask=STAGE_ALL, backward=False):
        return self.lib.mst_plan_launch_count(self.handle, mask, int(backward))

    def forward(self, mask, params, pitched, unpitched, ws=None):
        check(self.lib.mst_forward(self.handle, mask, ptr(params), ptr(self._touch(ws)), ptr(pitched),
                                   ptr(unpitched), current_stream(self.device)), 'mst_forward')

    def backward(self, mask, params, gparams, pitched, unpitched, ws=None):
        check(self.lib.mst_backward(self.handle, mask, ptr(params), ptr(gparams), ptr(self._touch(ws)),
                                    ptr(pitched), ptr(unpitched), current_stream(self.device)), 'mst_backward')

    def zero_grads(self, mask, ws=None):
        check(self.lib.mst_zero_grads(self.handle, mask, ptr(self.ws if ws is None else ws), current_stream(self.device)),
              'mst_zero_grads')

    def time_steps(self, mask, backward, params, gparams, pitched, unpitched, reps=20):
        import numpy as np
        n = self.lib.mst_plan_step_count(self.handle, mask, int(backward))
        ms, kind = np.zeros(n, np.float32), np.zeros(n, np.int32)
        fl, by = np.zeros(n, np.float64), np.zeros(n, np.float64)
        got = self.lib.mst_plan_time_steps(self.handle, mask, int(backward), ptr(params), ptr(gparams), ptr(self.ws),
                                           ptr(pitched), ptr(unpitched), current_stream(self.device), reps,
                                           ms.ctypes.data, kind.ctypes.data, fl.ctypes.data, by.ctypes.data)
        if got != n:
            check(got if got < 0 else -1, 'mst_plan_time_steps')
        return list(zip(kind.tolist(), ms.tolist(), fl.tolist(), by.tolist()))

    def step_carried(self, mask=STAGE_ALL, backward=False):
        import numpy as np
        n = self.lib.mst_plan_step_count(self.handle, mask, int(backward))
        out = np.zeros(n, np.int32)
        got = self.lib.mst_plan_step_carried(self.handle, mask, int(backward), out.ctypes.data)
        check(got if got < 0 else 0, 'mst_plan_step_carried')
        return out.tolist()

    def step_riders(self, mask=STAGE_ALL, backward=False):
        import numpy as np
        n = self.lib.mst_plan_step_count(self.handle, mask, int(backward))
        out = np.zeros(n, np.int32)
        got = self.lib.mst_plan_step_riders(self.handle, mask, int(backward), out.ctypes.data)
        check(got if got < 0 else 0, 'mst_plan_step_riders')
        return out.tolist()

    def zero_rides(self):
        got = self.lib.mst_plan_zero_rides(self.handle)
        check(got if got < 0 else 0, 'mst_plan_zero_rides')
        return got

    def step_gemms(self, mask, backward, step, cap=2048):
        import numpy as np
        out = np.zeros((cap, 6), np.int32)
        n = self.lib.mst_plan_step_gemms(self.handle, mask, int(backward), step, out.ctypes.data, cap)
        check(n if n < 0 else 0, 'mst_plan_step_gemms')
        return [tuple(r) for r in out[:n].tolist()]

    def tiled_train_iteration(self, params, gparams, pitched, unpitched, losses=None, is_root=True, all_reduce=None):
        if all_reduce is None:
            import torch.distributed as dist
            all_reduce = lambda t: dist.all_reduce(t, op=dist.ReduceOp.SUM)
        xoff, xlen, nx = (C.c_int64 * 8)(), (C.c_int64 * 8)(), C.c_int32()
        self._touch(None)
        for ph in range(self.lib.mst_tiled_phase_count(self.handle)):
            check(self.lib.mst_tiled_phase(self.handle, ph, ptr(params), ptr(gparams), ptr(self.ws), ptr(pitched), ptr(unpitched),
                                           ptr(losses), int(bool(is_root)), current_stream(self.device), C.byref(xoff), C.byref(xlen),
                                           C.byref(nx)), f'mst_tiled_phase({ph})')
            if nx.value == 1:
                all_reduce(self.ws[xoff[0]:xoff[0] + xlen[0]])
            elif nx.value > 1:
                parts = [self.ws[xoff[q]:xoff[q] + xlen[q]] for q in range(nx.value)]
                total = sum(int(xlen[q]) for q in range(nx.value))
                if getattr(self, '_xstage', None) is None or self._xstage.numel() < total:
                    self._xstage = torch.empty(total, dtype=torch.float32, device=self.device)
                stage = self._xstage[:total]
                torch.cat(parts, out=stage)
                all_reduce(stage)
                at = 0
                for t in parts:
                    t.copy_(stage[at:at + t.numel()])
                    at += t.numel()

    def train_iteration(self, params, gparams, pitched, unpitched, losses=None, ws=None):
        check(self.lib.mst_train_iteration(self.handle, ptr(params), ptr(gparams), ptr(self._touch(ws)),
                                           ptr(pitched), ptr(unpitched), ptr(losses), current_stream(self.device)),
              'mst_train_iteration')

    def eval_scratch(self):
        if getattr(self, '_eval_scratch', None) is None:
            n = self.lib.mst_eval_scratch_bytes(self.handle)
            if n <= 0:
                check(int(n) or -1, 'mst_eval_scratch_bytes')
            self._eval_scratch = torch.zeros(n // 8, dtype=torch.float64, device=self.device)
        return self._eval_scratch

    def eval_iteration(self, params, pitched, unpitched, losses, metrics, ws=None):
        if metrics.dtype != torch.float64 or not metrics.is_contiguous() or \
                metrics.numel() != self.clips * (self.dims.C + 2) * METRIC_WORDS:
            raise MstError('eval_iteration: metrics must be a contiguous float64 tensor of clips x (C + 2) x 8')
        check(self.lib.mst_eval_iteration(self.handle, ptr(params), ptr(self._touch(ws)), ptr(pitched), ptr(unpitched), ptr(losses),
                                          metrics.data_ptr(), self.eval_scratch().data_ptr(), current_stream(self.device)),
              'mst_eval_iteration')


_native = None


def get():
    global _native
    if _native is None:
        _native = Native()
    return _native
```

Baseline: 2751 iters/s.

## Add single-wave small-H LSTM kernels and ride LSTM backward inside GEMM launches

Adds single-wavefront LSTM forward and backward kernels for hidden sizes up to 16 that keep the recurrent weights in registers and stage the input projections through LDS. The planner also lets a small LSTM backward step ride as extra blocks inside a concurrent GEMM launch at the same level. The aim is to cut per-launch overhead and the waste of 256/1024-thread blocks on tiny recurrences. In exchange, the GEMM kernel gets another rider branch and uses more shared memory per block, and a slow LSTM rider can stretch the GEMM launch it is attached to.

```diff
diff --git a/__graft_entry__.py b/__graft_entry__.py
--- a/__graft_entry__.py
+++ b/__graft_entry__.py
@@ -27,7 +27,7 @@
 def build(force=False):
     os.makedirs(BUILD, exist_ok=True)
     hipcc = _hipcc()
-    headers = [os.path.join(CSRC, 'mst_common.h'), os.path.join(CSRC, 'combine_body.h'), os.path.join(ROOT, 'include', 'mst_amd.h')]
+    headers = [os.path.join(CSRC, 'mst_common.h'), os.path.join(CSRC, 'combine_body.h'), os.path.join(CSRC, 'lstm_small_body.h'), os.path.join(ROOT, 'include', 'mst_amd.h')]
     procs, objs = [], []
     for s in SOURCES:
         src, obj = os.path.join(CSRC, s + '.hip'), os.path.join(BUILD, s + '.o')
diff --git a/include/mst_amd.h b/include/mst_amd.h
--- a/include/mst_amd.h
+++ b/include/mst_amd.h
@@ -147,6 +147,8 @@
 int32_t mst_plan_step_carried(const mst_plan* p, int32_t stage_mask, int32_t backward, int32_t* carried);
 int32_t mst_plan_step_riders(const mst_plan* p, int32_t stage_mask, int32_t backward, int32_t* out);
 int32_t mst_plan_zero_rides(const mst_plan* p);
+int32_t mst_plan_step_carrier(const mst_plan* p, int32_t stage_mask, int32_t backward, int32_t* out);
+int32_t mst_plan_set_lstm_small(mst_plan* p, int32_t on);
 int32_t mst_plan_step_gemms(const mst_plan* p, int32_t stage_mask, int32_t backward, int32_t step, int32_t* out, int32_t cap);
 int32_t mst_plan_time_steps(const mst_plan* p, int32_t stage_mask, int32_t backward, const float* params,
                             float* gparams, float* ws, const float* pitched, const float* unpitched,
diff --git a/music-style-transfer_amd/csrc/gemm.hip b/music-style-transfer_amd/csrc/gemm.hip
--- a/music-style-transfer_amd/csrc/gemm.hip
+++ b/music-style-transfer_amd/csrc/gemm.hip
@@ -1,4 +1,5 @@
 #include "combine_body.h"
+#include "lstm_small_body.h"
 
 __device__ __forceinline__ float act_fwd(int act, float z, int col) {
     if (act == ACT_LEAKY) return z > 0.f ? z : z * LEAKY;
@@ -638,6 +639,17 @@
 __device__ __forceinline__ void segred_group(const SegRedDesc* __restrict__ descs, const int members, const int clip, const int lb, const int t, const Bases& b);
 
 __device__ __forceinline__ void gemm_rider_block(const GemmRiders& r, const int clip, int lb, const Bases& b, float* smem) {
+    const int lstm_blocks = r.lstm_members * r.lstm_blocks;
+    if (lb < lstm_blocks) {
+        const int m = lb / r.lstm_blocks, wave = MST_UNIFORM(threadIdx.x >> 6), bi = (lb - m * r.lstm_blocks) * (GEMM_THREADS / 64) + wave;
+        const LstmDesc d = r.lstms[clip * r.lstm_members + m];
+        if (bi >= d.B) return;
+        float* slice = smem + wave * LSTM_SW_LDS;
+        const int lane = threadIdx.x & 63;
+        lstm_small_bwd_body<LSTM_RIDE_H, true>(d, bi, lane, b, slice);
+        return;
+    }
+    lb -= lstm_blocks;
     const int seg_blocks = (r.seg_groups + 3) >> 2, gat_blocks = r.gat_members * r.gat_blocks;
 #pragma unroll
     for (int q = 0; q < 2; ++q) {
@@ -671,7 +683,7 @@
 
 __global__ __launch_bounds__(GEMM_THREADS) void gemm_kernel(const GemmDesc* __restrict__ descs, const int* __restrict__ owner, int count, int blocks_per_clip, int rider_blocks, Bases b, GemmRiders r) {
     constexpr int TILE_F = GEMM_BK * (GEMM_BM + GEMM_PAD), RED_F = (GEMM_THREADS / 64) * GEMM_BM * GEMM_BN;
-    __shared__ float smem[(2 * TILE_F > RED_F) ? 2 * TILE_F : RED_F];
+    __shared__ __attribute__((aligned(16))) float smem[(2 * TILE_F > RED_F) ? 2 * TILE_F : RED_F];
     float (*As)[GEMM_BM + GEMM_PAD] = reinterpret_cast<float (*)[GEMM_BM + GEMM_PAD]>(smem);
     float (*Bs)[GEMM_BN + GEMM_PAD] = reinterpret_cast<float (*)[GEMM_BN + GEMM_PAD]>(smem + TILE_F);
     const int clip = blockIdx.x / blocks_per_clip;
@@ -719,7 +731,7 @@
     return -1;
 }
 
-int gemm_rider_blocks(const GemmRiders& r) { return r.comb[0].sites * r.comb[0].blocks + r.comb[1].sites * r.comb[1].blocks + (r.seg_groups + 3) / 4 + r.gat_members * r.gat_blocks + r.zero_chunks; }
+int gemm_rider_blocks(const GemmRiders& r) { return r.lstm_members * r.lstm_blocks + r.comb[0].sites * r.comb[0].blocks + r.comb[1].sites * r.comb[1].blocks + (r.seg_groups + 3) / 4 + r.gat_members * r.gat_blocks + r.zero_chunks; }
 
 int launch_gemm(const GemmDesc* dev_descs, const int* dev_owner, int members, int blocks_per_clip, int clips, int mfma, Bases b, hipStream_t s, const GemmRiders* riders) {
     if (members <= 0 || blocks_per_clip <= 0 || clips <= 0) return 0;
diff --git a/music-style-transfer_amd/csrc/lstm.hip b/music-style-transfer_amd/csrc/lstm.hip
--- a/music-style-transfer_amd/csrc/lstm.hip
+++ b/music-style-transfer_amd/csrc/lstm.hip
@@ -1,17 +1,13 @@
 #include "mst_common.h"
+#include "lstm_small_body.h"
 
 #define LSTM_ZS 8192
 #define LSTM_MCH 32
-__device__ __forceinline__ float sigm(float x) { return MST_FAST_RCP(1.f + MST_FAST_EXP(-x)); }
-__device__ __forceinline__ float tanh_fast(float x) { return 2.f * sigm(2.f * x) - 1.f; }
 __device__ __forceinline__ float wsum(float v) {
 #pragma unroll
     for (int o = 32; o > 0; o >>= 1) v += __shfl_xor(v, o);
     return v;
 }
-
-typedef float lstm_f4 __attribute__((ext_vector_type(4)));
-typedef float lstm_f4u __attribute__((ext_vector_type(4), aligned(4)));
 
 template <bool REG>
 __global__ __launch_bounds__(REG ? 256 : 1024) void lstm_fwd_kernel(const LstmDesc* __restrict__ descs, Bases b) {
@@ -311,6 +307,21 @@
         MST_LDS_BARRIER();
     }
 #undef LSTM_LOAD
+}
+
+template <int KP>
+__global__ __launch_bounds__(64) void lstm_fwd_small_kernel(const LstmDesc* __restrict__ descs, Bases b) {
+    const LstmDesc d = descs[blockIdx.y];
+    if ((int)blockIdx.x >= d.B) return;
+    __shared__ __attribute__((aligned(16))) float lds[LSTM_SW_LDS];
+    lstm_small_fwd_body<KP>(d, blockIdx.x, threadIdx.x, b, lds);
+}
+template <int KP>
+__global__ __launch_bounds__(64) void lstm_bwd_small_kernel(const LstmDesc* __restrict__ descs, Bases b) {
+    const LstmDesc d = descs[blockIdx.y];
+    if ((int)blockIdx.x >= d.B) return;
+    __shared__ __attribute__((aligned(16))) float lds[LSTM_SW_LDS];
+    lstm_small_bwd_body<KP>(d, blockIdx.x, threadIdx.x, b, lds);
 }
 
 
@@ -735,11 +746,6 @@
     }
 }
 
-#ifdef HIPSIM
-#define LSTM_MULADD(a, b, c) ((a) * (b) + (c))
-#else
-#define LSTM_MULADD(a, b, c) __builtin_fmaf((a), (b), (c))
-#endif
 
 template <int N>
 __device__ __forceinline__ void gran_wait_joint(const lstm_gran_t* g, unsigned tag, int* status, bool& dead, float (&v)[N]) {
@@ -927,13 +933,24 @@
 static bool lstm_grouped(int count, int maxB) { return maxB >= 2 * LSTM_NS && (int64_t)count * maxB >= 2048; }
 #endif
 
-int launch_lstm_fwd(const LstmDesc* dev_descs, int count, int maxB, int maxH, int multi, Bases b, hipStream_t s) {
+bool lstm_small(int count, int maxB, int maxH) { return maxH <= LSTM_SH && !lstm_grouped(count, maxB); }
+#define LSTM_SMALL_LAUNCH(K)                                                                                         \
+    switch ((maxH + 3) / 4) {                                                                                        \
+    case 1: hipLaunchKernelGGL((K<4>), dim3(maxB, count), dim3(64), 0, s, dev_descs, b); break;                      \
+    case 2: hipLaunchKernelGGL((K<8>), dim3(maxB, count), dim3(64), 0, s, dev_descs, b); break;                      \
+    case 3: hipLaunchKernelGGL((K<12>), dim3(maxB, count), dim3(64), 0, s, dev_descs, b); break;                     \
+    default: hipLaunchKernelGGL((K<16>), dim3(maxB, count), dim3(64), 0, s, dev_descs, b); break;                    \
+    }
+
+int launch_lstm_fwd(const LstmDesc* dev_descs, int count, int maxB, int maxH, int multi, int small, Bases b, hipStream_t s) {
     if (count <= 0) return 0;
     if (multi) {
         MST_LAUNCH_CORESIDENT(lstm_multi_fwd_kernel, dim3(LSTM_NB, count), dim3(256), s, dev_descs, b);
         return (int)hipGetLastError();
     }
-    if (maxH <= 64 && lstm_grouped(count, maxB))
+    if (small && lstm_small(count, maxB, maxH)) {
+        LSTM_SMALL_LAUNCH(lstm_fwd_small_kernel)
+    } else if (maxH <= 64 && lstm_grouped(count, maxB))
         hipLaunchKernelGGL(lstm_fwd_group_kernel, dim3((maxB + LSTM_NS - 1) / LSTM_NS, count), dim3(256), 0, s, dev_descs, b);
     else if (maxH <= 64)
         hipLaunchKernelGGL((lstm_fwd_kernel<true>), dim3(maxB, count), dim3(block_for(maxH)), 0, s, dev_descs, b);
@@ -944,13 +961,15 @@
     return (int)hipGetLastError();
 }
 
-int launch_lstm_bwd(const LstmDesc* dev_descs, int count, int maxB, int maxH, int multi, Bases b, hipStream_t s) {
+int launch_lstm_bwd(const LstmDesc* dev_descs, int count, int maxB, int maxH, int multi, int small, Bases b, hipStream_t s) {
     if (count <= 0) return 0;
     if (multi) {
         MST_LAUNCH_CORESIDENT(lstm_multi_bwd_kernel, dim3(LSTM_NB, count), dim3(256), s, dev_descs, b);
         return (int)hipGetLastError();
     }
-    if (maxH <= 64 && lstm_grouped(count, maxB))
+    if (small && lstm_small(count, maxB, maxH)) {
+        LSTM_SMALL_LAUNCH(lstm_bwd_small_kernel)
+    } else if (maxH <= 64 && lstm_grouped(count, maxB))
         hipLaunchKernelGGL(lstm_bwd_group_kernel, dim3((maxB + LSTM_NS - 1) / LSTM_NS, count), dim3(256), 0, s, dev_descs, b);
     else if (maxH <= 64)
         hipLaunchKernelGGL((lstm_bwd_kernel<true>), dim3(maxB, count), dim3(block_for(maxH)), 0, s, dev_descs, b);
diff --git a/music-style-transfer_amd/csrc/lstm_small_body.h b/music-style-transfer_amd/csrc/lstm_small_body.h
--- /dev/null
+++ b/music-style-transfer_amd/csrc/lstm_small_body.h
@@ -0,0 +1,272 @@
+#pragma once
+#include "mst_common.h"
+
+__device__ __forceinline__ float sigm(float x) { return MST_FAST_RCP(1.f + MST_FAST_EXP(-x)); }
+__device__ __forceinline__ float tanh_fast(float x) { return 2.f * sigm(2.f * x) - 1.f; }
+
+typedef float lstm_f4 __attribute__((ext_vector_type(4)));
+typedef float lstm_f4u __attribute__((ext_vector_type(4), aligned(4)));
+
+
+#define LSTM_SH 16
+#define LSTM_SW_X 64
+#define LSTM_SW_LDS 1024
+#ifdef HIPSIM
+#define LSTM_MULADD(a, b, c) ((a) * (b) + (c))
+#else
+#define LSTM_MULADD(a, b, c) __builtin_fmaf((a), (b), (c))
+#endif
+__device__ __forceinline__ float lstm_cell_update(const float fg, const float c, const float ig, const float gg) {
+#pragma clang fp contract(off)
+    const float keep = fg * c, add = ig * gg;
+    return keep + add;
+}
+
+#define LSTM_WL_F(KP) (4 * (KP) * (KP))
+template <int KP, bool BWD>
+__device__ __forceinline__ void lstm_small_stage_whh(const MST_GLOBAL_AS float* whh, const int H, const int u, float* w_s) {
+    constexpr int N = LSTM_WL_F(KP) / 64;
+#pragma unroll
+    for (int i = 0; i < N; ++i) w_s[u + 64 * i] = 0.f;
+    MST_WAVE_SYNC();
+    const int total = 4 * H * H, dq = 64 / H, dr = 64 - dq * H;
+    float t[N];
+#pragma unroll
+    for (int i = 0; i < N; ++i) t[i] = whh[min(u + 64 * i, total - 1)];
+    int row = u / H, col = u - row * H;
+#pragma unroll
+    for (int i = 0; i < N; ++i) {
+        const int g = (row >= H) + (row >= 2 * H) + (row >= 3 * H), rr = row - g * H;
+        if (u + 64 * i < total) w_s[BWD ? (g * KP + rr) * KP + col : (g * KP + col) * KP + rr] = t[i];
+        row += dq; col += dr;
+        if (col >= H) { col -= H; ++row; }
+    }
+}
+
+template <int KP, bool WL = false>
+__device__ __forceinline__ void lstm_small_fwd_body(const LstmDesc& d, const int bi, const int u, const Bases& b, float* lds) {
+    const int H = d.H, G = 4 * d.H;
+    float* x_s = lds;
+    float* w_s = lds + LSTM_SW_X;
+    float* zx_s = lds + LSTM_SW_X + (WL ? LSTM_WL_F(KP) : 0);
+    const int zchunk = (LSTM_SW_LDS - LSTM_SW_X - (WL ? LSTM_WL_F(KP) : 0)) / G;
+    const MST_GLOBAL_AS float* whh = (const MST_GLOBAL_AS float*)(b.p[SP_PAR] + d.whh_off);
+    const MST_GLOBAL_AS float* bhh = (const MST_GLOBAL_AS float*)(b.p[SP_PAR] + d.bhh_off);
+    const MST_GLOBAL_AS float* zx = (const MST_GLOBAL_AS float*)(b.p[SP_WS] + d.zx_off) + (int64_t)bi * d.S * G;
+    MST_GLOBAL_AS float* ws = (MST_GLOBAL_AS float*)b.p[SP_WS];
+    MST_GLOBAL_AS float* tmp = (MST_GLOBAL_AS float*)b.p[SP_TMP];
+    lstm_f4u wv[WL ? 1 : 4][WL ? 1 : KP / 4];
+    const int wlast = max(G * H - 4, 0);
+    const int uc = min(u, H - 1);
+    if constexpr (!WL) {
+#pragma unroll
+        for (int q = 0; q < 4; ++q) {
+#pragma unroll
+            for (int k4 = 0; k4 < KP / 4; ++k4)
+                wv[q][k4] = *reinterpret_cast<const MST_GLOBAL_AS lstm_f4u*>(whh + min((q * H + uc) * H + 4 * k4, wlast));
+        }
+    }
+    float bias[4];
+#pragma unroll
+    for (int q = 0; q < 4; ++q) bias[q] = bhh[q * H + uc];
+    constexpr int NT = 16;
+    auto fetch = [&](const int step) {
+        const int cnt = min(zchunk, d.S - step);
+        if (u < G) {
+            const int sstep = d.reverse ? -G : G;
+            const MST_GLOBAL_AS float* zg = zx + (int64_t)(d.reverse ? d.S - 1 - step : step) * G + u;
+            for (int i0 = 0; i0 < cnt; i0 += NT) {
+                float t[NT];
+#pragma unroll
+                for (int i = 0; i < NT; ++i) t[i] = zg[(int64_t)min(i0 + i, cnt - 1) * sstep];
+#pragma unroll
+                for (int i = 0; i < NT; ++i) MST_PIN(t[i]);
+#pragma unroll
+                for (int i = 0; i < NT; ++i) {
+                    if (i0 + i < cnt) zx_s[(i0 + i) * G + u] = t[i];
+                }
+            }
+        }
+    };
+    fetch(0);
+    x_s[u] = 0.f;
+    if constexpr (WL) lstm_small_stage_whh<KP, false>(whh, H, u, w_s);
+#pragma unroll
+    for (int q = 0; q < 4; ++q) MST_PIN(bias[q]);
+    float w[WL ? 1 : 4][WL ? 1 : KP];
+#pragma unroll
+    for (int q = 0; q < (WL ? 0 : 4); ++q) {
+#pragma unroll
+        for (int k4 = 0; k4 < KP / 4; ++k4) {
+            const int flat = (q * H + uc) * H + 4 * k4, sh = flat - min(flat, wlast);
+            const lstm_f4u r = wv[q][k4];
+            float v0 = r.x, v1 = r.y, v2 = r.z;
+            v0 = sh == 1 ? r.y : v0; v0 = sh == 2 ? r.z : v0; v0 = sh == 3 ? r.w : v0;
+            v1 = sh == 1 ? r.z : v1; v1 = sh == 2 ? r.w : v1;
+            v2 = sh == 1 ? r.w : v2;
+            w[q][4 * k4] = 4 * k4 < H ? v0 : 0.f; w[q][4 * k4 + 1] = 4 * k4 + 1 < H ? v1 : 0.f;
+            w[q][4 * k4 + 2] = 4 * k4 + 2 < H ? v2 : 0.f; w[q][4 * k4 + 3] = 4 * k4 + 3 < H ? r.w : 0.f;
+        }
+    }
+    float c = 0.f, hown = 0.f;
+    int slot = 0;
+    const int rstep = d.reverse ? -1 : 1;
+    int64_t row = (int64_t)bi * d.S + (d.reverse ? d.S - 1 : 0);
+    for (int step = 0; step < d.S; ++step, ++slot, row += rstep) {
+        if (slot == zchunk) {
+            MST_WAVE_SYNC();
+            fetch(step);
+            slot = 0;
+        }
+        MST_WAVE_SYNC();
+        float hv[KP], zq[4];
+#pragma unroll
+        for (int k = 0; k < KP; ++k) hv[k] = x_s[k];
+#pragma unroll
+        for (int q = 0; q < 4; ++q) zq[q] = zx_s[slot * G + q * H + uc];
+        MST_WAVE_SYNC();
+        if (u < H) {
+            float a[4];
+#pragma unroll
+            for (int q = 0; q < 4; ++q) {
+                float z[4] = {0.f, 0.f, 0.f, 0.f};
+                if constexpr (WL) {
+                    float wq[KP];
+#pragma unroll
+                    for (int k = 0; k < KP; ++k) wq[k] = w_s[(q * KP + k) * KP + u];
+#pragma unroll
+                    for (int k = 0; k < KP; k += 4) {
+#pragma unroll
+                        for (int r = 0; r < 4; ++r) z[r] = fmaf(wq[k + r], hv[k + r], z[r]);
+                    }
+                    __builtin_amdgcn_sched_barrier(0);
+                } else {
+#pragma unroll
+                    for (int k = 0; k < KP; k += 4) {
+#pragma unroll
+                        for (int r = 0; r < 4; ++r) z[r] = fmaf(w[q][k + r], hv[k + r], z[r]);
+                    }
+                }
+                a[q] = (((z[0] + z[1]) + (z[2] + z[3])) + zq[q]) + bias[q];
+            }
+            const float ig = sigm(a[0]), fg = sigm(a[1]), gg = tanh_fast(a[2]), og = sigm(a[3]);
+            c = lstm_cell_update(fg, c, ig, gg);
+            const float tc = tanh_fast(c);
+            const float h = og * tc;
+            x_s[u] = h;
+            tmp[d.hprev_off + row * H + u] = hown;
+            tmp[d.tc_off + row * H + u] = tc;
+            MST_GLOBAL_AS float* g = tmp + d.gates_off + row * G;
+            g[u] = ig; g[H + u] = fg; g[2 * H + u] = gg; g[3 * H + u] = og;
+            tmp[d.c_off + row * H + u] = c;
+            ws[d.out_off + row * d.out_ld + u] = h;
+            hown = h;
+        }
+    }
+}
+
+template <int KP, bool WL = false>
+__device__ __forceinline__ void lstm_small_bwd_body(const LstmDesc& d, const int bi, const int u, const Bases& b, float* lds) {
+    const int H = d.H, G = 4 * d.H;
+    float* dz_s = lds;
+    float* w_s = lds + LSTM_SW_X;
+    float* sv_s = lds + LSTM_SW_X + (WL ? LSTM_WL_F(KP) : 0);
+    const int schunk = (LSTM_SW_LDS - LSTM_SW_X - (WL ? LSTM_WL_F(KP) : 0)) / (7 * H);
+    const MST_GLOBAL_AS float* whh = (const MST_GLOBAL_AS float*)(b.p[SP_PAR] + d.whh_off);
+    const MST_GLOBAL_AS float* tmp = (const MST_GLOBAL_AS float*)b.p[SP_TMP];
+    MST_GLOBAL_AS float* gr = (MST_GLOBAL_AS float*)b.p[SP_GRAD];
+    const int uc = min(u, H - 1);
+    float w[WL ? 1 : 4][WL ? 1 : KP];
+#pragma unroll
+    for (int p = 0; p < (WL ? 0 : 4); ++p) {
+#pragma unroll
+        for (int jj = 0; jj < KP; ++jj) {
+            const float v = whh[(p * H + min(jj, H - 1)) * H + uc];
+            w[p][jj] = jj < H ? v : 0.f;
+        }
+    }
+    const int ku = u & 15, kq = u >> 4;
+    auto stage = [&](const int step) {
+        const int cnt = min(schunk, step + 1);
+        if (ku < H) {
+#pragma unroll(WL ? 2 : 4)
+            for (int i = kq; i < cnt; i += 4) {
+                const int st = step - i;
+                const int s_ = d.reverse ? d.S - 1 - st : st, sp_ = d.reverse ? s_ + 1 : s_ - 1;
+                const int64_t row_ = (int64_t)bi * d.S + s_;
+                const MST_GLOBAL_AS float* g_ = tmp + d.gates_off + row_ * G;
+                float t[7];
+                t[0] = g_[ku]; t[1] = g_[H + ku]; t[2] = g_[2 * H + ku]; t[3] = g_[3 * H + ku];
+                t[4] = tmp[d.tc_off + row_ * H + ku];
+                const float cp = tmp[d.c_off + ((int64_t)bi * d.S + (st > 0 ? sp_ : s_)) * H + ku];
+                t[5] = st > 0 ? cp : 0.f;
+                t[6] = gr[d.gout_off + row_ * d.out_ld + ku];
+#pragma unroll
+                for (int q = 0; q < 7; ++q) sv_s[(i * 7 + q) * H + ku] = t[q];
+            }
+        }
+    };
+    stage(d.S - 1);
+    dz_s[u] = 0.f;
+    if constexpr (WL) lstm_small_stage_whh<KP, true>(whh, H, u, w_s);
+#pragma unroll
+    for (int p = 0; p < (WL ? 0 : 4); ++p) {
+#pragma unroll
+        for (int jj = 0; jj < KP; ++jj) MST_PIN(w[p][jj]);
+    }
+    float dc_next = 0.f, red[4] = {0.f, 0.f, 0.f, 0.f};
+    int slot = 0;
+    const int rstep = d.reverse ? 1 : -1;
+    int64_t row = (int64_t)bi * d.S + (d.reverse ? 0 : d.S - 1);
+    for (int step = d.S - 1; step >= 0; --step, ++slot, row += rstep) {
+        if (slot == schunk) {
+            MST_WAVE_SYNC();
+            stage(step);
+            slot = 0;
+        }
+        MST_WAVE_SYNC();
+        if (u < H) {
+            float sv[7];
+#pragma unroll
+            for (int q = 0; q < 7; ++q) sv[q] = sv_s[(slot * 7 + q) * H + u];
+            const float ig = sv[0], fg = sv[1], gg = sv[2], og = sv[3], tc = sv[4], cprev = sv[5];
+            const float dh = sv[6] + ((red[0] + red[1]) + (red[2] + red[3]));
+            const float dc = LSTM_MULADD(dh * og, LSTM_MULADD(-tc, tc, 1.f), dc_next);
+            const float dzi = dc * gg * ig * (1.f - ig);
+            const float dzf = dc * cprev * fg * (1.f - fg);
+            const float dzg = dc * ig * LSTM_MULADD(-gg, gg, 1.f);
+            const float dzo = dh * tc * og * (1.f - og);
+            dc_next = dc * fg;
+            dz_s[u] = dzi; dz_s[16 + u] = dzf; dz_s[32 + u] = dzg; dz_s[48 + u] = dzo;
+            MST_GLOBAL_AS float* gz = gr + d.gzx_off + row * G;
+            gz[u] = dzi; gz[H + u] = dzf; gz[2 * H + u] = dzg; gz[3 * H + u] = dzo;
+        }
+        if (step == 0) break;
+        MST_WAVE_SYNC();
+#pragma unroll
+        for (int p = 0; p < 4; ++p) {
+            float dv[KP];
+#pragma unroll
+            for (int jj = 0; jj < KP; ++jj) dv[jj] = dz_s[16 * p + jj];
+            float a[4] = {0.f, 0.f, 0.f, 0.f};
+            if constexpr (WL) {
+                float wp[KP];
+#pragma unroll
+                for (int jj = 0; jj < KP; ++jj) wp[jj] = w_s[(p * KP + jj) * KP + uc];
+#pragma unroll
+                for (int jj = 0; jj < KP; jj += 4) {
+#pragma unroll
+                    for (int r = 0; r < 4; ++r) a[r] = fmaf(wp[jj + r], dv[jj + r], a[r]);
+                }
+                __builtin_amdgcn_sched_barrier(0);
+            } else {
+#pragma unroll
+                for (int jj = 0; jj < KP; jj += 4) {
+#pragma unroll
+                    for (int r = 0; r < 4; ++r) a[r] = fmaf(w[p][jj + r], dv[jj + r], a[r]);
+                }
+            }
+            red[p] = (a[0] + a[1]) + (a[2] + a[3]);
+        }
+    }
+}
diff --git a/music-style-transfer_amd/csrc/mst_common.h b/music-style-transfer_amd/csrc/mst_common.h
--- a/music-style-transfer_amd/csrc/mst_common.h
+++ b/music-style-transfer_amd/csrc/mst_common.h
@@ -133,7 +133,9 @@
     const GatherDesc* gathers; int32_t gat_members, gat_blocks;
     struct Comb { const CombineDesc* descs; int32_t sites, blocks, kind; } comb[2];
     const ZeroChunk* zero; int32_t zero_chunks; int64_t zero_stride;
-};
+    const struct LstmDesc* lstms; int32_t lstm_members, lstm_blocks;
+};
+#define LSTM_RIDE_H 8
 
 struct LstmDesc {
     int32_t B, S, H, reverse;
@@ -284,8 +286,9 @@
 int launch_segred(const SegRedDesc* dev_descs, int members, int blocks_per_clip, int clips, int stage2_blocks, Bases b, hipStream_t s);
 int launch_segred2(const SegRedDesc* dev_descs, int count, int stage2_blocks, Bases b, hipStream_t s);
 int launch_lstm_transpose(const LstmDesc* dev_descs, int count, int maxH, int multi, Bases b, hipStream_t s);
-int launch_lstm_fwd(const LstmDesc* dev_descs, int count, int maxB, int maxH, int multi, Bases b, hipStream_t s);
-int launch_lstm_bwd(const LstmDesc* dev_descs, int count, int maxB, int maxH, int multi, Bases b, hipStream_t s);
+int launch_lstm_fwd(const LstmDesc* dev_descs, int count, int maxB, int maxH, int multi, int small, Bases b, hipStream_t s);
+int launch_lstm_bwd(const LstmDesc* dev_descs, int count, int maxB, int maxH, int multi, int small, Bases b, hipStream_t s);
+bool lstm_small(int count, int maxB, int maxH);
 int lstm_multi_blocks_per_cu();
 int launch_combine_fwd(const CombineDesc* dev_descs, int count, int max_nblk, int all_small, int mc4, Bases b, hipStream_t s);
 int launch_combine_bwd(const CombineDesc* dev_descs, int count, int max_nblk, int all_small, int mc4, Bases b, hipStream_t s);
diff --git a/music-style-transfer_amd/csrc/plan.hip b/music-style-transfer_amd/csrc/plan.hip
--- a/music-style-transfer_amd/csrc/plan.hip
+++ b/music-style-transfer_amd/csrc/plan.hip
@@ -221,7 +221,8 @@
 };
 
 struct CombRide { int first = 0, sites = 0, nblk = 0, bwd = 0; };
-struct Riders { int seg_first = 0, seg_members = 0, seg_groups = 0, seg_stage2 = 0, gat_first = 0, gat_members = 0, gat_rows = 0; CombRide comb[2]; };
+struct Riders { int seg_first = 0, seg_members = 0, seg_groups = 0, seg_stage2 = 0, gat_first = 0, gat_members = 0, gat_rows = 0; CombRide comb[2];
+                int lstm_first = 0, lstm_members = 0, lstm_maxB = 0; };
 struct Step { int kind, first, count, a, b, stage; int c = 0; int lvl = 0; int chain = -1; int signal = -1; int wait[3] = {-1, -1, -1};
               int carried = 0; Riders ride; };
 struct Acc { int space; int64_t lo, hi; bool w; bool accum = false, dense = true; };
@@ -253,6 +254,7 @@
     int err = 0;
     mst_plan_options opt{};
     int mfma = 0;
+    int lstm_small_on = 1;
 
     bool tiled() const { return opt.tile_rows > 0; }
     bool mixes() const { return !mfma && !tiled() && opt.branches != 1 && !opt.no_merge; }
@@ -1356,7 +1358,9 @@
         if (!mixes()) continue;
         for (size_t e = lv_begin; e < out.size(); ++e) {
             const bool comb = (out[e].kind == K_COMB_F || out[e].kind == K_COMB_B) && mc4();
-            if (out[e].kind != K_GATHER && out[e].kind != K_SEGRED && !comb) continue;
+            const bool lstm = out[e].kind == K_LSTM_B && out[e].b <= LSTM_RIDE_H &&
+                              lstm_small(out[e].count, out[e].a, out[e].b);
+            if (out[e].kind != K_GATHER && out[e].kind != K_SEGRED && !comb && !lstm) continue;
             for (size_t c = lv_begin; c < out.size(); ++c) {
                 Step& g = out[c];
                 if (g.kind != K_GEMM || (!across_stages && g.stage != out[e].stage)) continue;
@@ -1364,6 +1368,7 @@
                 if (s.kind == K_GATHER && !g.ride.gat_members) { g.ride.gat_first = s.first; g.ride.gat_members = s.count / K(); g.ride.gat_rows = s.a; }
                 else if (s.kind == K_SEGRED && !g.ride.seg_members) { g.ride.seg_first = s.first; g.ride.seg_members = s.count / K(); g.ride.seg_groups = s.a; g.ride.seg_stage2 = s.b; }
                 else if (comb && !g.ride.comb[s.b != 0].sites) g.ride.comb[s.b != 0] = CombRide{s.first, s.count / K(), s.a, s.kind == K_COMB_B};
+                else if (lstm && !g.ride.lstm_members) { g.ride.lstm_first = s.first; g.ride.lstm_members = s.count / K(); g.ride.lstm_maxB = s.a; }
                 else continue;
                 out[e].carried = 1;
                 break;
@@ -1730,6 +1735,8 @@
             r.comb[large] = {p->combines.dev + c.first, c.sites, large ? (c.nblk + 3) / 4 : 1,
                              large ? (c.bwd ? COMB_RIDE_REDUCE : COMB_RIDE_SUMSQ) : (c.bwd ? COMB_RIDE_SMALL_B : COMB_RIDE_SMALL_F)};
         }
+        if (q.lstm_members) { r.lstms = p->lstms.dev + q.lstm_first; r.lstm_members = q.lstm_members; r.lstm_blocks = (q.lstm_maxB + GEMM_THREADS / 64 - 1) / (GEMM_THREADS / 64);
+}
         if (with_zero) { r.zero = p->d_zero_all; r.zero_chunks = (int)p->zero_all.size(); r.zero_stride = p->act_top; }
         int e = launch_gemm(p->gemms.dev + s.first, p->d_gemm_owner + s.c, s.b, s.a, clips, p->mfma, b, st, &r);
         if (!e) e = launch_segred2(p->segreds.dev + q.seg_first, q.seg_members * clips, q.seg_stage2, b, st);
@@ -1740,8 +1747,8 @@
     case K_GATHER: return launch_gather(p->gathers.dev + s.first, s.count, s.a, b, st);
     case K_SEGRED: return launch_segred(p->segreds.dev + s.first, s.count / p->K(), s.a, p->K(), s.b, b, st);
     case K_LSTM_T: return launch_lstm_transpose(p->lstms.dev + s.first, s.count, s.b, p->lstms.sched[s.first].multi, b, st);
-    case K_LSTM_F: return launch_lstm_fwd(p->lstms.dev + s.first, s.count, s.a, s.b, p->lstms.sched[s.first].multi, b, st);
-    case K_LSTM_B: return launch_lstm_bwd(p->lstms.dev + s.first, s.count, s.a, s.b, p->lstms.sched[s.first].multi, b, st);
+    case K_LSTM_F: return launch_lstm_fwd(p->lstms.dev + s.first, s.count, s.a, s.b, p->lstms.sched[s.first].multi, p->lstm_small_on, b, st);
+    case K_LSTM_B: return launch_lstm_bwd(p->lstms.dev + s.first, s.count, s.a, s.b, p->lstms.sched[s.first].multi, p->lstm_small_on, b, st);
     case K_COMB_F: return launch_combine_fwd(p->combines.dev + s.first, s.count, s.a, s.b == 0 ? (p->mc4() ? 2 : 1) : 0, p->mc4(), b, st);
     case K_COMB_B: return launch_combine_bwd(p->combines.dev + s.first, s.count, s.a, s.b == 0 ? (p->mc4() ? 2 : 1) : 0, p->mc4(), b, st);
     case K_COMB_F1: return launch_combine_phase(p->combines.dev + s.first, s.a, 0, b, st, 1, p->mc4());
@@ -2106,9 +2113,46 @@
     for (auto& s : p->list(mask, backward)) {
         if (!(s.stage & mask)) continue;
         const bool two = (s.kind == K_SEGRED && s.b > 0) || ((s.kind == K_COMB_F || s.kind == K_COMB_B) && s.b != 0);
-        out[n++] = !s.carried ? 0 : (two ? 2 : 1);
+        out[n++] = (!s.carried || s.kind == K_LSTM_F || s.kind == K_LSTM_B) ? 0 : (two ? 2 : 1);
     }
     return n;
+}
+
+extern "C" int32_t mst_plan_step_carrier(const mst_plan* p, int32_t mask, int32_t backward, int32_t* out) {
+    if (!p || !out) return MST_ERR_ARG;
+    const std::vector<Step>& L = p->list(mask, backward);
+    std::vector<int> pos(L.size(), -1);
+    int n = 0;
+    for (size_t i = 0; i < L.size(); ++i) if (L[i].stage & mask) pos[i] = n++;
+    for (size_t i = 0; i < L.size(); ++i) {
+        const Step& s = L[i];
+        if (pos[i] < 0) continue;
+        int at = -1;
+        if (s.carried)
+            for (size_t c = 0; c < L.size() && at < 0; ++c) {
+                const Step& g = L[c];
+                if (g.kind != K_GEMM || g.lvl != s.lvl) continue;
+                const Riders& q = g.ride;
+                const bool mine = (s.kind == K_GATHER && q.gat_members && q.gat_first == s.first) ||
+                                  (s.kind == K_SEGRED && q.seg_members && q.seg_first == s.first) ||
+                                  ((s.kind == K_COMB_F || s.kind == K_COMB_B) && q.comb[s.b != 0].sites && q.comb[s.b != 0].first == s.first &&
+                                   q.comb[s.b != 0].bwd == (s.kind == K_COMB_B)) ||
+                                  (s.kind == K_LSTM_B && q.lstm_members && q.lstm_first == s.first);
+                if (mine) at = pos[c];
+            }
+        out[pos[i]] = at;
+    }
+    return n;
+}
+
+extern "C" int32_t mst_plan_set_lstm_small(mst_plan* p, int32_t on) {
+    if (!p) return MST_ERR_ARG;
+    for (int pass = 0; pass < 2; ++pass)
+        for (const std::vector<Step>* L : {&p->sched[pass], &p->sched_all[pass]})
+            for (const Step& s : *L)
+                if ((s.kind == K_LSTM_F || s.kind == K_LSTM_B) && s.carried) return MST_ERR_UNSUPPORTED;
+    p->lstm_small_on = on ? 1 : 0;
+    return MST_OK;
 }
 
 extern "C" int32_t mst_plan_zero_rides(const mst_plan* p) { return !p ? MST_ERR_ARG : (p->zero_ride >= 0 ? 1 : 0); }
diff --git a/music-style-transfer_amd/style/_native.py b/music-style-transfer_amd/style/_native.py
--- a/music-style-transfer_amd/style/_native.py
+++ b/music-style-transfer_amd/style/_native.py
@@ -117,6 +117,8 @@
     'mst_plan_step_carried': (C.c_int32, [_P, C.c_int32, C.c_int32, _P]),
     'mst_plan_step_riders': (C.c_int32, [_P, C.c_int32, C.c_int32, _P]),
     'mst_plan_zero_rides': (C.c_int32, [_P]),
+    'mst_plan_step_carrier': (C.c_int32, [_P, C.c_int32, C.c_int32, _P]),
+    'mst_plan_set_lstm_small': (C.c_int32, [_P, C.c_int32]),
     'mst_plan_step_gemms': (C.c_int32, [_P, C.c_int32, C.c_int32, C.c_int32, _P, C.c_int32]),
     'mst_plan_time_steps': (C.c_int32, [_P, C.c_int32, C.c_int32, _P, _P, _P, _P, _P, _P, C.c_int32, _P, _P, _P, _P]),
     'mst_audio_plan_create': (_P, [C.c_int32, C.c_int32, C.c_int64, C.POINTER(C.c_int32)]),
@@ -364,6 +366,17 @@
         got = self.lib.mst_plan_step_riders(self.handle, mask, int(backward), out.ctypes.data)
         check(got if got < 0 else 0, 'mst_plan_step_riders')
         return out.tolist()
+
+    def step_carrier(self, mask=STAGE_ALL, backward=False):
+        import numpy as np
+        n = self.lib.mst_plan_step_count(self.handle, mask, int(backward))
+        out = np.zeros(n, np.int32)
+        got = self.lib.mst_plan_step_carrier(self.handle, mask, int(backward), out.ctypes.data)
+        check(got if got < 0 else 0, 'mst_plan_step_carrier')
+        return out.tolist()
+
+    def set_lstm_small(self, on):
+        check(self.lib.mst_plan_set_lstm_small(self.handle, int(on)), 'mst_plan_set_lstm_small')
 
     def zero_rides(self):
         got = self.lib.mst_plan_zero_rides(self.handle)
```

New measurement: 2852 iters/s (median of 6 runs). 3.7% higher.
